# jorge-menjivar/tekken-rs

Hardware: AMD Instinct MI355X
Metric: input MB/s tokenized (whole node) (higher is better)
Workload: dtype u8

## Files before the change

include/tekken_hip.h:

```cpp
#ifndef TEKKEN_HIP_H
#define TEKKEN_HIP_H
#include <stddef.h>
#include <stdint.h>

#ifdef __cplusplus
extern "C" {
#endif

#define TK_OK 0
#define TK_ERR_INVALID_CONFIG (-1)
#define TK_ERR_RUNTIME (-2)
#define TK_ERR_INVALID_UTF8 (-3)
#define TK_ERR_NO_DEVICE (-4)
#define TK_ERR_INVALID_ARG (-5)
#define TK_ERR_IO (-6)
#define TK_ERR_JSON (-7)
#define TK_ERR_BASE64 (-8)
#define TK_ERR_TOKEN_NOT_FOUND (-9)
#define TK_ERR_SPECIAL_POLICY (-10)

#define TK_POLICY_IGNORE 0
#define TK_POLICY_KEEP 1
#define TK_POLICY_RAISE 2

typedef struct tk_ctx tk_ctx;


int tk_ctx_create(const uint8_t* token_bytes, const uint32_t* token_offsets, uint32_t n_ranks,
                  uint32_t num_special_tokens, uint32_t bos_id, uint32_t eos_id, int device_id,
                  tk_ctx** out_ctx);

void tk_ctx_destroy(tk_ctx* ctx);

const char* tk_last_error(const tk_ctx* ctx);

typedef struct tk_result {
    uint32_t* ids;
    uint64_t* offsets;
    uint64_t n_ids;
    uint64_t n_docs;
} tk_result;

int tk_encode_batch(tk_ctx* ctx, const uint8_t* bytes, const uint64_t* doc_offsets, uint64_t n_docs,
                    int add_bos, int add_eos, int validate_utf8, tk_result* out);
void tk_free_result(tk_result* r);

int tk_encode_one(tk_ctx* ctx, const uint8_t* text, uint64_t len, int add_bos, int add_eos, uint32_t* ids_out,
                  uint64_t ids_capacity, uint64_t* n_ids);
uint64_t tk_small_path_calls(const tk_ctx* ctx);
uint64_t tk_round_path_docs(const tk_ctx* ctx);
uint64_t tk_long_piece_records(const tk_ctx* ctx);
uint64_t tk_cut_chunks(const tk_ctx* ctx);
uint64_t tk_last_host_syncs(const tk_ctx* ctx);

int tk_ctx_set_memo(tk_ctx* ctx, int log2_entries, int policy);
int tk_ctx_memo_clear(tk_ctx* ctx);
int tk_memo_stats(const tk_ctx* ctx, uint64_t* lookups_last, uint64_t* hits_last, uint64_t* lookups_total, uint64_t* hits_total,
                  int* active_last);

int tk_ctx_set_pattern(tk_ctx* ctx, int mode);

void* tk_host_alloc(size_t bytes);
void tk_host_free(void* p);
int tk_encode_batch_pipelined(tk_ctx* ctx, const uint8_t* bytes, const uint64_t* doc_offsets, uint64_t n_docs,
                              int add_bos, int add_eos, uint64_t slice_bytes, uint32_t* ids_out, uint64_t ids_capacity,
                              uint64_t* offsets_out, uint64_t* n_ids);

int tk_encode_batch_device(tk_ctx* ctx, const void* d_bytes, const void* d_doc_offsets, uint64_t n_docs,
                           uint64_t n_bytes, int add_bos, int add_eos, void* hip_stream, void** d_ids,
                           void** d_out_offsets, uint64_t* n_ids);

#define TK_CHECK_OFFSETS 1
#define TK_CHECK_UTF8 2
int tk_encode_batch_device_ex(tk_ctx* ctx, const void* d_bytes, const void* d_doc_offsets, uint64_t n_docs, uint64_t n_bytes,
                              int add_bos, int add_eos, int checks, void* hip_stream, void** d_ids, void** d_out_offsets,
                              uint64_t* n_ids);

#define TK_SPANS_CHECK_COVER 4
#define TK_SPANS_CHECK_BYTES 8
int tk_token_spans_device(tk_ctx* ctx, const void* d_ids, const void* d_id_offsets, uint64_t n_docs, uint64_t n_ids,
                          const void* d_doc_offsets, const void* d_bytes, int checks, void* hip_stream, void** d_spans,
                          uint64_t* bad_doc);
int tk_encode_batch_device_spans(tk_ctx* ctx, const void* d_bytes, const void* d_doc_offsets, uint64_t n_docs, uint64_t n_bytes,
                                 int add_bos, int add_eos, int checks, void* hip_stream, void** d_ids, void** d_out_offsets,
                                 void** d_spans, uint64_t* n_ids, uint64_t* bad_doc);
int tk_encode_batch_spans(tk_ctx* ctx, const uint8_t* bytes, const uint64_t* doc_offsets, uint64_t n_docs, int add_bos,
                          int add_eos, int validate_utf8, int checks, tk_result* out, uint32_t** spans, uint64_t* bad_doc);
void tk_free_spans(uint32_t* spans);

#define TK_UNIT_BYTE 0
#define TK_UNIT_CHAR 1
#define TK_UNIT_UTF16 2
int tk_token_spans_units_device(tk_ctx* ctx, const void* d_ids, const void* d_id_offsets, uint64_t n_docs, uint64_t n_ids, int unit,
                                void* hip_stream, void** d_spans);
int tk_encode_batch_device_spans_units(tk_ctx* ctx, const void* d_bytes, const void* d_doc_offsets, uint64_t n_docs, uint64_t n_bytes,
                                       int add_bos, int add_eos, int checks, int unit, void* hip_stream, void** d_ids,
                                       void** d_out_offsets, void** d_spans, uint64_t* n_ids);
int tk_encode_batch_spans_units(tk_ctx* ctx, const uint8_t* bytes, const uint64_t* doc_offsets, uint64_t n_docs, int add_bos,
                                int add_eos, int validate_utf8, int unit, tk_result* out, uint32_t** spans);
int tk_spans_locate_device(tk_ctx* ctx, const void* d_spans, const void* d_id_offsets, uint64_t n_docs, uint64_t n_ids,
                           const void* d_ann_doc, const void* d_ann, uint64_t n_ann, void* hip_stream, void** d_tok_range,
                           uint64_t* bad_ann);

#define TK_DENSE_PAD_LEFT 1
#define TK_DENSE_TRUNC_LEFT 2
#define TK_DENSE_FIXED 4
#define TK_DENSE_I64 8
#define TK_DENSE_MASK 16
typedef struct tk_dense_opts { uint32_t max_length, multiple_of, pad_id, keep_head, keep_tail, flags; } tk_dense_opts;
typedef struct tk_dense { void* ids; uint8_t* mask; uint32_t* lengths; uint64_t n_docs, row_len, n_truncated; } tk_dense;
int tk_dense_from_ids_device(tk_ctx* ctx, const void* d_ids, const void* d_id_offsets, uint64_t n_docs, uint64_t n_ids,
                             const tk_dense_opts* opts, void* hip_stream, tk_dense* out);
int tk_encode_batch_device_dense(tk_ctx* ctx, const void* d_bytes, const void* d_doc_offsets, uint64_t n_docs, uint64_t n_bytes,
                                 int add_bos, int add_eos, int checks, const tk_dense_opts* opts, void* hip_stream,
                                 void** d_ids, void** d_out_offsets, uint64_t* n_ids, tk_dense* out);
int tk_encode_batch_dense(tk_ctx* ctx, const uint8_t* bytes, const uint64_t* doc_offsets, uint64_t n_docs, int add_bos,
                          int add_eos, int validate_utf8, const tk_dense_opts* opts, tk_dense* out);
void tk_free_dense(tk_dense* out);
int tk_ragged_from_dense_device(tk_ctx* ctx, const void* d_dense, uint64_t n_docs, uint64_t row_len, int flags,
                                const void* d_lengths, uint32_t pad_id, void* hip_stream, void** d_ids,
                                void** d_id_offsets, uint64_t* n_ids);

#define TK_SEQPACK_I64 1
#define TK_SEQPACK_POSITIONS 2
#define TK_SEQPACK_SEGMENTS 4
#define TK_SEQPACK_CU_SEQLENS 8
#define TK_SEQPACK_DROP_LAST 16
typedef struct tk_seqpack_opts { uint32_t seq_len, pad_id, flags; } tk_seqpack_opts;
typedef struct tk_seqpack { void *input_ids, *position_ids, *segment_ids; int32_t* cu_seqlens;
                            uint64_t n_rows, row_len, n_used, n_left, n_segments, max_seqlen; } tk_seqpack;
int tk_seqpack_from_ids_device(tk_ctx* ctx, const void* d_ids, const void* d_id_offsets, uint64_t n_docs, uint64_t n_ids,
                               const tk_seqpack_opts* opts, void* hip_stream, tk_seqpack* out);
int tk_encode_batch_device_seqpack(tk_ctx* ctx, const void* d_bytes, const void* d_doc_offsets, uint64_t n_docs, uint64_t n_bytes,
                                   int add_bos, int add_eos, int checks, const tk_seqpack_opts* opts, void* hip_stream,
                                   void** d_ids, void** d_out_offsets, uint64_t* n_ids, tk_seqpack* out);
int tk_encode_batch_seqpack(tk_ctx* ctx, const uint8_t* bytes, const uint64_t* doc_offsets, uint64_t n_docs, int add_bos, int add_eos,
// ... 172 lines not shown
```

tekken-rs_amd/__init__.py:

```python
import ctypes
import enum
import os
import subprocess

import numpy as np

_HERE = os.path.dirname(os.path.abspath(__file__))
LIB_PATH = os.environ.get("TK_HIP_LIB") or os.path.join(_HERE, "libtekken_hip.so")
INCLUDE_DIR = os.path.join(os.path.dirname(_HERE), "include")

TK_OK = 0
CHECK_OFFSETS, CHECK_UTF8 = 1, 2
SPANS_CHECK_COVER, SPANS_CHECK_BYTES = 4, 8
UNIT_BYTE, UNIT_CHAR, UNIT_UTF16 = 0, 1, 2
_UNITS = {"byte": UNIT_BYTE, "char": UNIT_CHAR, "utf16": UNIT_UTF16}
DENSE_PAD_LEFT, DENSE_TRUNC_LEFT, DENSE_FIXED, DENSE_I64, DENSE_MASK = 1, 2, 4, 8, 16
SEQPACK_I64, SEQPACK_POSITIONS, SEQPACK_SEGMENTS, SEQPACK_CU_SEQLENS, SEQPACK_DROP_LAST = 1, 2, 4, 8, 16
WINDOW_FIXED, WINDOW_I64, WINDOW_MASK, WINDOW_SPANS = 1, 2, 4, 8
CHECK_PARTS = 16
JOIN_NONE = 0xFFFFFFFF
PART_LABEL_CTRL, PART_LABEL_TEXT = 1, 2
JOIN_LABELS, JOIN_PART_INDEX = 1, 2
ROWFIT_I64, ROWFIT_POSITIONS, ROWFIT_SEGMENTS, ROWFIT_CU_SEQLENS, ROWFIT_LABELS, ROWFIT_DOC_START = 1, 2, 4, 8, 16, 32
REGROUP_ORDER_KEEP, REGROUP_ORDER_LENGTH, REGROUP_ORDER_SHUFFLE, REGROUP_ORDER_GROUPED = 0, 1, 2, 3
# ... 76 lines not shown

class _Join(ctypes.Structure):
    _fields_ = [("ids", ctypes.c_void_p), ("offsets", ctypes.c_void_p), ("labels", ctypes.c_void_p), ("part_index", ctypes.c_void_p),
                ("n_convs", ctypes.c_uint64), ("n_parts", ctypes.c_uint64), ("n_ids", ctypes.c_uint64), ("n_ctrl", ctypes.c_uint64),
                ("n_labelled", ctypes.c_uint64)]


class _RowfitOpts(ctypes.Structure):
    _fields_ = [("seq_len", ctypes.c_uint32), ("pad_id", ctypes.c_uint32), ("keep_tail", ctypes.c_uint32), ("flags", ctypes.c_uint32),
                ("ignore_index", ctypes.c_int32)]


class _Rowfit(ctypes.Structure):
    _fields_ = [("input_ids", ctypes.c_void_p), ("labels", ctypes.c_void_p), ("position_ids", ctypes.c_void_p), ("segment_ids", ctypes.c_void_p),
                ("cu_seqlens", ctypes.c_void_p), ("doc_start", ctypes.c_void_p), ("n_rows", ctypes.c_uint64), ("row_len", ctypes.c_uint64),
                ("n_segments", ctypes.c_uint64), ("max_seqlen", ctypes.c_uint64), ("n_truncated", ctypes.c_uint64), ("n_pad", ctypes.c_uint64)]


class _RegroupOpts(ctypes.Structure):
    _fields_ = [("max_tokens", ctypes.c_uint64), ("min_length", ctypes.c_uint32), ("max_length", ctypes.c_uint32), ("order", ctypes.c_uint32),
                ("seed", ctypes.c_uint32), ("window", ctypes.c_uint32), ("max_docs", ctypes.c_uint32), ("flags", ctypes.c_uint32)]


class _Regroup(ctypes.Structure):
    _fields_ = [("ids", ctypes.c_void_p), ("offsets", ctypes.c_void_p), ("labels", ctypes.c_void_p), ("perm", ctypes.c_void_p),
                ("batch_offsets", ctypes.c_void_p), ("batch_rowlen", ctypes.c_void_p), ("n_docs", ctypes.c_uint64), ("n_ids", ctypes.c_uint64),
                ("n_masked", ctypes.c_uint64), ("n_short", ctypes.c_uint64), ("n_long", ctypes.c_uint64), ("n_batches", ctypes.c_uint64),
                ("n_oversize", ctypes.c_uint64), ("n_batch_pad", ctypes.c_uint64)]


_LIB = None


def build(force=False):
    if force:
        subprocess.check_call(["make", "-s", "-C", _HERE, "clean"])
    subprocess.check_call(["make", "-s", "-j4", "-C", _HERE, "libtekken_hip.so"])
    return LIB_PATH


def lib():
    global _LIB
    if _LIB is not None:
        return _LIB
    if not os.path.exists(LIB_PATH):
        raise RuntimeError("libtekken_hip.so is missing: run `make -C tekken-rs_amd` (or __graft_entry__.build())")
    try:
        import torch
    except ImportError:
        pass
    L = ctypes.CDLL(LIB_PATH)
    vp, u8p, u32p, u64p = ctypes.c_void_p, ctypes.POINTER(ctypes.c_uint8), ctypes.POINTER(ctypes.c_uint32), ctypes.POINTER(ctypes.c_uint64)
    L.tk_ctx_create.restype = ctypes.c_int
    L.tk_ctx_create.argtypes = [u8p, u32p, ctypes.c_uint32, ctypes.c_uint32, ctypes.c_uint32, ctypes.c_uint32,
                                ctypes.c_int, ctypes.POINTER(vp)]
    L.tk_ctx_destroy.argtypes = [vp]
    L.tk_last_error.restype = ctypes.c_char_p
    L.tk_last_error.argtypes = [vp]
    L.tk_encode_batch.restype = ctypes.c_int
    L.tk_encode_batch.argtypes = [vp, u8p, u64p, ctypes.c_uint64, ctypes.c_int, ctypes.c_int, ctypes.c_int,
                                  ctypes.POINTER(_Result)]
    L.tk_free_result.argtypes = [ctypes.POINTER(_Result)]
    L.tk_encode_one.restype = ctypes.c_int
    L.tk_encode_one.argtypes = [vp, ctypes.c_char_p, ctypes.c_uint64, ctypes.c_int, ctypes.c_int, u32p, ctypes.c_uint64, u64p]
    L.tk_small_path_calls.restype = ctypes.c_uint64
    L.tk_small_path_calls.argtypes = [vp]
    L.tk_round_path_docs.restype = ctypes.c_uint64
    L.tk_round_path_docs.argtypes = [vp]
    L.tk_long_piece_records.restype = ctypes.c_uint64
    L.tk_long_piece_records.argtypes = [vp]
    if hasattr(L, "tk_ctx_set_memo"):
        L.tk_ctx_set_memo.restype = ctypes.c_int
        L.tk_ctx_set_memo.argtypes = [vp, ctypes.c_int, ctypes.c_int]
        L.tk_ctx_memo_clear.restype = ctypes.c_int
        L.tk_ctx_memo_clear.argtypes = [vp]
        L.tk_memo_stats.restype = ctypes.c_int
        L.tk_memo_stats.argtypes = [vp, u64p, u64p, u64p, u64p, ctypes.POINTER(ctypes.c_int)]
    if hasattr(L, "tk_last_host_syncs"):
        L.tk_last_host_syncs.restype = ctypes.c_uint64
        L.tk_last_host_syncs.argtypes = [vp]
    if hasattr(L, "tk_cut_chunks"):
        L.tk_cut_chunks.restype = ctypes.c_uint64
        L.tk_cut_chunks.argtypes = [vp]
    L.tk_encode_batch_device.restype = ctypes.c_int
    L.tk_encode_batch_device.argtypes = [vp, vp, vp, ctypes.c_uint64, ctypes.c_uint64, ctypes.c_int, ctypes.c_int, vp,
                                         ctypes.POINTER(vp), ctypes.POINTER(vp), ctypes.POINTER(ctypes.c_uint64)]
    L.tk_encode_batch_device_ex.restype = ctypes.c_int
    L.tk_encode_batch_device_ex.argtypes = [vp, vp, vp, ctypes.c_uint64, ctypes.c_uint64, ctypes.c_int, ctypes.c_int, ctypes.c_int, vp,
                                            ctypes.POINTER(vp), ctypes.POINTER(vp), ctypes.POINTER(ctypes.c_uint64)]
    L.tk_host_alloc.restype = ctypes.c_void_p
    L.tk_host_alloc.argtypes = [ctypes.c_size_t]
    L.tk_host_free.argtypes = [ctypes.c_void_p]
    L.tk_encode_batch_pipelined.restype = ctypes.c_int
    L.tk_encode_batch_pipelined.argtypes = [vp, u8p, u64p, ctypes.c_uint64, ctypes.c_int, ctypes.c_int, ctypes.c_uint64, u32p,
                                            ctypes.c_uint64, u64p, u64p]
    L.tk_ids18_bytes.restype = ctypes.c_uint64
    L.tk_ids18_bytes.argtypes = [ctypes.c_uint64]
    L.tk_pack_ids18_device.restype = ctypes.c_int
    L.tk_pack_ids18_device.argtypes = [vp, vp, ctypes.c_uint64, vp, vp]
    L.tk_unpack_ids18_device.restype = ctypes.c_int
    L.tk_unpack_ids18_device.argtypes = [vp, vp, ctypes.c_uint64, vp, vp]
    L.tk_ctx_set_pattern.restype = ctypes.c_int
    L.tk_ctx_set_pattern.argtypes = [vp, ctypes.c_int]
    L.tk_tokenizer_set_honour_pattern.restype = ctypes.c_int
    L.tk_tokenizer_set_honour_pattern.argtypes = [vp, ctypes.c_int]
    L.tk_ctx_set_special_tokens.restype = ctypes.c_int
    L.tk_ctx_set_special_tokens.argtypes = [vp, u8p, u32p, ctypes.c_uint32]
    L.tk_decode_batch.restype = ctypes.c_int
    L.tk_decode_batch.argtypes = [vp, u32p, u64p, ctypes.c_uint64, ctypes.c_int, ctypes.POINTER(_TextResult), u64p]
    L.tk_free_text_result.argtypes = [ctypes.POINTER(_TextResult)]
    L.tk_decode_batch_device.restype = ctypes.c_int
    L.tk_decode_batch_device.argtypes = [vp, vp, vp, ctypes.c_uint64, ctypes.c_uint64, ctypes.c_int, vp, ctypes.POINTER(vp),
                                         ctypes.POINTER(vp), u64p, u64p]
    L.tk_tokenizer_decode_batch.restype = ctypes.c_int
    L.tk_tokenizer_decode_batch.argtypes = [vp, u32p, u64p, ctypes.c_uint64, ctypes.c_int, ctypes.POINTER(_TextResult), u64p]
    L.tk_last_timing.restype = ctypes.c_int
    if hasattr(L, "tk_last_merge_ms"):
        L.tk_last_merge_ms.restype = ctypes.c_float
        L.tk_last_merge_ms.argtypes = [vp]
    L.tk_last_timing.argtypes = [vp, ctypes.POINTER(ctypes.c_float), ctypes.POINTER(ctypes.c_float)]
    L.tk_last_stats.restype = ctypes.c_int
    L.tk_last_stats.argtypes = [vp, u64p, u64p]
    L.tk_split_batch.restype = ctypes.c_int
    L.tk_split_batch.argtypes = [vp, u8p, u64p, ctypes.c_uint64, u8p]
    L.tk_tokenizer_from_file.restype = ctypes.c_int
    L.tk_tokenizer_from_file.argtypes = [ctypes.c_char_p, ctypes.c_int, ctypes.POINTER(vp)]
    L.tk_tokenizer_from_json.restype = ctypes.c_int
    L.tk_tokenizer_from_json.argtypes = [ctypes.c_char_p, ctypes.c_size_t, ctypes.c_int, ctypes.POINTER(vp)]
    L.tk_tokenizer_destroy.argtypes = [vp]
    L.tk_tokenizer_last_error.restype = ctypes.c_char_p
    L.tk_tokenizer_last_error.argtypes = [vp]
    L.tk_tokenizer_encode.restype = ctypes.c_int
    L.tk_tokenizer_encode.argtypes = [vp, ctypes.c_char_p, ctypes.c_size_t, ctypes.c_int, ctypes.c_int,
                                      ctypes.POINTER(u32p), ctypes.POINTER(ctypes.c_size_t)]
    L.tk_tokenizer_encode_batch.restype = ctypes.c_int
    L.tk_tokenizer_encode_batch.argtypes = [vp, u8p, u64p, ctypes.c_uint64, ctypes.c_int, ctypes.c_int,
                                            ctypes.POINTER(_Result)]
    L.tk_free_ids.argtypes = [u32p]
    L.tk_tokenizer_decode.restype = ctypes.c_int
    L.tk_tokenizer_decode.argtypes = [vp, u32p, ctypes.c_size_t, ctypes.c_int, ctypes.POINTER(ctypes.c_void_p),
                                      ctypes.POINTER(ctypes.c_size_t)]
    L.tk_free_text.argtypes = [ctypes.c_void_p]
    u64pp = ctypes.POINTER(ctypes.POINTER(ctypes.c_uint64))
    L.tk_free_offsets.argtypes = [ctypes.POINTER(ctypes.c_uint64)]
    L.tk_free_offsets.restype = None
    L.tk_tokenizer_decode_all.restype = ctypes.c_int
    L.tk_tokenizer_decode_all.argtypes = [vp, u32p, ctypes.c_size_t, ctypes.c_int, ctypes.POINTER(ctypes.c_void_p), u64pp,
                                          ctypes.POINTER(ctypes.c_size_t)]
    L.tk_tokenizer_vocab.restype = ctypes.c_int
    L.tk_tokenizer_vocab.argtypes = [vp, ctypes.POINTER(ctypes.c_void_p), u64pp, ctypes.POINTER(ctypes.c_size_t)]
    L.tk_tokenizer_vocab_size.restype = ctypes.c_uint32
    L.tk_tokenizer_vocab_size.argtypes = [vp]
    L.tk_tokenizer_num_special_tokens.restype = ctypes.c_uint32
    L.tk_tokenizer_num_special_tokens.argtypes = [vp]
    L.tk_tokenizer_version.restype = ctypes.c_char_p
    L.tk_tokenizer_version.argtypes = [vp]
    L.tk_tokenizer_control_token.restype = ctypes.c_int
    L.tk_tokenizer_control_token.argtypes = [vp, ctypes.c_char_p, u32p]
    L.tk_tokenizer_is_special.restype = ctypes.c_int
    L.tk_tokenizer_is_special.argtypes = [vp, ctypes.c_uint32]
    L.tk_tokenizer_is_byte.restype = ctypes.c_int
    L.tk_tokenizer_is_byte.argtypes = [vp, ctypes.c_uint32]
    L.tk_tokenizer_id_to_piece.restype = ctypes.c_int
    L.tk_tokenizer_id_to_piece.argtypes = [vp, ctypes.c_uint32, ctypes.POINTER(ctypes.c_void_p),
                                           ctypes.POINTER(ctypes.c_size_t)]
    L.tk_tokenizer_id_to_byte_piece.restype = ctypes.c_int
# ... 637 lines not shown
        return JoinResult.take(j)[1]

    def ragged_from_dense_device(self, d_dense_ptr, n_docs, row_len, flags=0, d_lengths_ptr=0, pad_id=0, stream=0):
        d_ids, d_oo, n = ctypes.c_void_p(), ctypes.c_void_p(), ctypes.c_uint64(0)
        self._call("tk_ragged_from_dense_device", ctypes.c_void_p(d_dense_ptr or None), n_docs, row_len, int(flags),
                   ctypes.c_void_p(d_lengths_ptr or None), int(pad_id), ctypes.c_void_p(stream),
                   ctypes.byref(d_ids), ctypes.byref(d_oo), ctypes.byref(n))
        return d_ids.value, d_oo.value, int(n.value)

    def encode_batch_device_views(self, d_bytes_ptr, d_offs_ptr, n_docs, n_bytes, add_bos=True, add_eos=True, stream=0):
        p_ids, p_oo, n = self.encode_batch_device(d_bytes_ptr, d_offs_ptr, n_docs, n_bytes, add_bos, add_eos, stream)
        return DeviceView(p_ids, n, "<i4"), DeviceView(p_oo, n_docs + 1, "<i8")

    def pack_ids18_device(self, d_ids_ptr, n_ids, d_packed_ptr, stream=0):
        rc = lib().tk_pack_ids18_device(self._h, ctypes.c_void_p(d_ids_ptr), n_ids, ctypes.c_void_p(d_packed_ptr), ctypes.c_void_p(stream))
        if rc != TK_OK:
            raise self._err(rc)

    def unpack_ids18_device(self, d_packed_ptr, n_ids, d_ids_ptr, stream=0):
        rc = lib().tk_unpack_ids18_device(self._h, ctypes.c_void_p(d_packed_ptr), n_ids, ctypes.c_void_p(d_ids_ptr), ctypes.c_void_p(stream))
        if rc != TK_OK:
            raise self._err(rc)

    def set_pattern(self, mode):
        rc = lib().tk_ctx_set_pattern(self._h, int(mode))
        if rc != TK_OK:
            raise self._err(rc)

    def set_special_tokens(self, strings):
        raw = [x.encode("utf-8") if isinstance(x, str) else bytes(x) for x in strings]
        offs = np.zeros(len(raw) + 1, np.uint32)
        offs[1:] = np.cumsum([len(x) for x in raw], dtype=np.uint64).astype(np.uint32)
        blob = np.frombuffer(b"".join(raw) or b"\0", dtype=np.uint8).copy()
        rc = lib().tk_ctx_set_special_tokens(self._h, _p(blob, ctypes.c_uint8), _p(offs, ctypes.c_uint32), len(raw))
        if rc != TK_OK:
            raise self._err(rc)

    def decode_batch(self, ids, offs, policy=SpecialTokenPolicy.Ignore):
        ids = np.ascontiguousarray(ids, dtype=np.uint32)
        offs = np.ascontiguousarray(offs, dtype=np.uint64)
        res = _TextResult()
        bad = ctypes.c_uint64(0)
        ibuf = ids if len(ids) else np.zeros(1, np.uint32)
        rc = lib().tk_decode_batch(self._h, _p(ibuf, ctypes.c_uint32), _p(offs, ctypes.c_uint64), len(offs) - 1, int(policy),
                                   ctypes.byref(res), ctypes.byref(bad))
        if rc != TK_OK:
            e = self._err(rc)
            e.bad_doc = int(bad.value)
            raise e
        n, D = int(res.n_bytes), int(res.n_docs)
        data = np.ctypeslib.as_array(res.bytes, shape=(max(n, 1),))[:n].copy()
        oo = np.ctypeslib.as_array(res.offsets, shape=(D + 1,)).copy()
        lib().tk_free_text_result(ctypes.byref(res))
        return data, oo

    def decode_docs(self, id_lists, policy=SpecialTokenPolicy.Ignore):
        offs = np.zeros(len(id_lists) + 1, np.uint64)
        if id_lists:
            offs[1:] = np.cumsum([len(x) for x in id_lists], dtype=np.uint64)
        ids = np.array([i for x in id_lists for i in x], dtype=np.uint32)
        data, oo = self.decode_batch(ids, offs, policy)
        raw = data.tobytes()
        return [raw[int(oo[d]):int(oo[d + 1])] for d in range(len(id_lists))]

    def decode_batch_device(self, d_ids_ptr, d_offs_ptr, n_docs, n_ids, policy=SpecialTokenPolicy.Ignore, stream=0):
        d_b, d_o, n, bad = ctypes.c_void_p(), ctypes.c_void_p(), ctypes.c_uint64(0), ctypes.c_uint64(0)
        rc = lib().tk_decode_batch_device(self._h, ctypes.c_void_p(d_ids_ptr), ctypes.c_void_p(d_offs_ptr), n_docs, n_ids,
                                          int(policy), ctypes.c_void_p(stream), ctypes.byref(d_b), ctypes.byref(d_o),
                                          ctypes.byref(n), ctypes.byref(bad))
        if rc != TK_OK:
            e = self._err(rc)
            e.bad_doc = int(bad.value)
            raise e
        return DeviceView(d_b.value, int(n.value), "|u1"), DeviceView(d_o.value, n_docs + 1, "<i8")

    def last_timing(self):
        a, b = ctypes.c_float(0), ctypes.c_float(0)
        lib().tk_last_timing(self._h, ctypes.byref(a), ctypes.byref(b))
        return {"pipeline_ms": a.value, "encode_kernel_ms": b.value, "merge_ms": float(lib().tk_last_merge_ms(self._h)) if hasattr(lib(), "tk_last_merge_ms") else 0.0}

    def last_stats(self):
        a, b = ctypes.c_uint64(0), ctypes.c_uint64(0)
        lib().tk_last_stats(self._h, ctypes.byref(a), ctypes.byref(b))
        return {"long_docs": int(a.value), "handed_back": int(b.value)}

    def split_docs(self, docs):
        data, offs = pack_docs(docs)
        n = int(offs[-1])
        out = np.zeros(max(n, 1), np.uint8)
        dbuf = data if n else np.zeros(1, np.uint8)
        rc = lib().tk_split_batch(self._h, _p(dbuf, ctypes.c_uint8), _p(offs, ctypes.c_uint64), len(docs),
                                  _p(out, ctypes.c_uint8))
        if rc != TK_OK:
            raise self._err(rc)
        res = []
        for d in range(len(docs)):
            a, b = int(offs[d]), int(offs[d + 1])
            res.append(np.nonzero(out[a:b])[0].tolist())
        return res


class Node:

    def __init__(self, token_bytes, num_special, bos_id, eos_id, devices=(0,)):
        toks = list(token_bytes)
        offs = np.zeros(len(toks) + 1, np.uint32)
        offs[1:] = np.cumsum([len(t) for t in toks], dtype=np.uint64).astype(np.uint32)
        blob = np.frombuffer(b"".join(toks) or b"\0", dtype=np.uint8)
        devs = (ctypes.c_int * len(devices))(*devices)
        h = ctypes.c_void_p()
        rc = lib().tk_node_create(_p(blob, ctypes.c_uint8), _p(offs, ctypes.c_uint32), len(toks), num_special, bos_id, eos_id,
                                  devs, len(devices), ctypes.byref(h))
        if rc != TK_OK:
            raise TokenizerError(rc, lib().tk_node_last_error(None).decode())
        self._h = h

    def close(self):
        if getattr(self, "_h", None):
            lib().tk_node_destroy(self._h)
            self._h = None

    def __del__(self):
        try:
            self.close()
        except Exception:
            pass

    def n_devices(self):
        return lib().tk_node_n_devices(self._h)

    def encode_batch(self, data, offs, add_bos=True, add_eos=True):
        data = np.ascontiguousarray(data, dtype=np.uint8)
        offs = np.ascontiguousarray(offs, dtype=np.uint64)
        res = _Result()
        dbuf = data if len(data) else np.zeros(1, np.uint8)
        rc = lib().tk_node_encode_batch(self._h, _p(dbuf, ctypes.c_uint8), _p(offs, ctypes.c_uint64), len(offs) - 1, int(add_bos),
                                        int(add_eos), ctypes.byref(res))
        if rc != TK_OK:
            raise TokenizerError(rc, lib().tk_node_last_error(self._h).decode())
        return _take_result(res)

    def encode_batch_into(self, data, offs, ids_out, offs_out, add_bos=True, add_eos=True):
        assert data.dtype == np.uint8 and offs.dtype == np.uint64 and ids_out.dtype == np.uint32 and offs_out.dtype == np.uint64
        assert len(offs_out) >= len(offs), "offs_out holds %d offsets, the call writes %d" % (len(offs_out), len(offs))
        for a in (data, offs, ids_out, offs_out):
            assert a.flags["C_CONTIGUOUS"], "tk_node_encode_batch_pinned wants contiguous buffers"
        n = ctypes.c_uint64(0)
        dbuf = data if len(data) else np.zeros(1, np.uint8)
        rc = lib().tk_node_encode_batch_pinned(self._h, _p(dbuf, ctypes.c_uint8), _p(offs, ctypes.c_uint64), len(offs) - 1, int(add_bos),
                                               int(add_eos), _p(ids_out, ctypes.c_uint32), len(ids_out), _p(offs_out, ctypes.c_uint64), ctypes.byref(n))
        if rc != TK_OK:
            raise TokenizerError(rc, lib().tk_node_last_error(self._h).decode())
        return int(n.value)

    def last_timing(self):
        a, b = ctypes.c_float(0), ctypes.c_float(0)
        lib().tk_node_last_timing(self._h, ctypes.byref(a), ctypes.byref(b))
        return {"kernels_ms_max": a.value, "gather_ms": b.value}

    def last_shards(self):
        n = self.n_devices()
        b, i = (ctypes.c_uint64 * n)(), (ctypes.c_uint64 * n)()
        lib().tk_node_last_shards(self._h, b, i, n)
        return list(b), list(i)


class _Pinned:
# ... 547 lines not shown
```

tekken-rs_amd/csrc/tk_capi.cpp:

```cpp
#include <unordered_map>

#include "tk_ctx.h"

static thread_local std::string g_tls_err;

void tk_set_tls_error(const std::string& e) { g_tls_err = e; }
const std::string& tk_get_tls_error() { return g_tls_err; }

namespace {

struct PinPool {
    std::mutex mu;
    std::unordered_map<void*, size_t> live;
    std::vector<std::pair<void*, size_t>> free_blocks;
    size_t free_bytes = 0;
    void* get(size_t bytes) {
        if (bytes == 0) bytes = 1;
        {
            std::lock_guard<std::mutex> lock(mu);
            size_t best = free_blocks.size();
            for (size_t i = 0; i < free_blocks.size(); ++i)
                if (free_blocks[i].second >= bytes && free_blocks[i].second <= 4 * bytes + (1u << 16) &&
                    (best == free_blocks.size() || free_blocks[i].second < free_blocks[best].second))
                    best = i;
// ... 29 lines not shown
                }
            }
        }
        (void)hipHostFree(p);
    }
};
PinPool g_pin_pool;

}

void* tk_pinned_get(size_t bytes) { return g_pin_pool.get(bytes); }
void tk_pinned_put(void* p) { g_pin_pool.put(p); }

int upload(tk_ctx* c, DevBuf& b, const void* src, size_t bytes) {
    TK_HIP(c, b.reserve(bytes ? bytes : 16));
    if (bytes) TK_HIP(c, hipMemcpy(b.p, src, bytes, hipMemcpyHostToDevice));
    return TK_OK;
}

int check_n_docs(tk_ctx* c, uint64_t n_docs) {
    if (n_docs >= 0xFFFFFFF0ull) { c->err = "too many documents in one batch"; return TK_ERR_INVALID_ARG; }
    return TK_OK;
}
int enter_device(tk_ctx* c, uint64_t n_docs) {
    int rc = check_n_docs(c, n_docs);
    if (rc != TK_OK) return rc;
    TK_HIP(c, hipSetDevice(c->device));
    return TK_OK;
}

static int copy_out_fail(tk_ctx* c, CopyOut* a, int n, const std::string& err) {
    for (int i = 0; i < n; ++i) { tk_pinned_put(a[i].host); a[i].host = nullptr; }
    c->err = err;
    return TK_ERR_RUNTIME;
}
int pinned_blocks(tk_ctx* c, CopyOut* a, int n) {
    bool ok = true;
    for (int i = 0; i < n; ++i)
        if (a[i].selected) ok = (a[i].host = tk_pinned_get(a[i].bytes)) != nullptr && ok;
    return ok ? TK_OK : copy_out_fail(c, a, n, "hipHostMalloc failed");
}
int copy_out(tk_ctx* c, CopyOut* a, int n, const char* what) {
    int rc = pinned_blocks(c, a, n);
    if (rc != TK_OK) return rc;
    hipError_t e = hipSuccess;
    for (int i = 0; i < n && e == hipSuccess; ++i)
        if (a[i].selected && a[i].dev && a[i].bytes) e = hipMemcpyAsync(a[i].host, a[i].dev, a[i].bytes, hipMemcpyDeviceToHost, c->stream);
    if (e == hipSuccess) e = hipStreamSynchronize(c->stream);
    return e == hipSuccess ? TK_OK : copy_out_fail(c, a, n, std::string(what) + " copy failed: " + hipGetErrorString(e));
}

int check_flags_and_args(tk_ctx* c, int checks, int known, bool null_arg) {
    if (checks & ~known) { c->err = "unknown check flag"; return TK_ERR_INVALID_ARG; }
    if (null_arg) { c->err = "null argument"; return TK_ERR_INVALID_ARG; }
    return TK_OK;
}
int scan_u32(tk_ctx* c, DevBuf& workspace, const uint32_t* counts, uint64_t n, uint64_t* offs, hipStream_t s) {
    TK_HIP(c, workspace.reserve(scan_workspace_bytes(n)));
    TK_HIP(c, tk_launch_scan(counts, n, offs, (uint64_t*)workspace.p, s));
    return TK_OK;
}
int encode_batch_for_layout(tk_ctx* c, const uint8_t* bytes, const uint64_t* doc_offsets, uint64_t n_docs, int add_bos, int add_eos,
                            int validate_utf8, DevBatch* dev, uint64_t* n_ids) {
    tk_result res;
    int rc = encode_batch(c, bytes, doc_offsets, n_docs, add_bos, add_eos, validate_utf8, &res, dev);
    if (rc != TK_OK) return rc;
    *n_ids = res.n_ids;
    tk_free_result(&res);
    return TK_OK;
}

static void read_knobs(TkKnobs& k) {
    if (const char* tl = getenv("TK_TAIL")) k.serial_tail = strcmp(tl, "serial") == 0;
    if (const char* dg = getenv("TK_DECODE_GROUPS")) k.no_decode_groups = strcmp(dg, "0") == 0;
    if (const char* gl = getenv("TK_DECODE_GROUP_LIMIT")) { const long long v = atoll(gl); if (v > 0 && v < 0x7FFFFF00ll) k.decode_group_limit = (uint32_t)v; }
    if (const char* fl = getenv("TK_FLAT_LONG")) k.no_flat_long = atoi(fl) == 0;
    if (const char* fl = getenv("TK_FLAT_LONG128")) k.no_flat_long128 = atoi(fl) == 0;
    if (const char* fl = getenv("TK_FLAT_CUT")) k.no_flat_cut = atoi(fl) == 0;
    if (const char* lm = getenv("TK_LONG_MIN")) k.long_min = (uint32_t)atoi(lm);
    if (const char* lz = getenv("TK_LONG_LAZY_MUL")) k.long_lazy_mul = (uint32_t)atoi(lz);
    if (const char* lf = getenv("TK_LONG_FORCE")) k.long_force = (uint32_t)atoi(lf);
    if (const char* ml = getenv("TK_MEMO_LOG2")) { const int v = atoi(ml); k.memo_log2 = v <= 0 ? 0u : (uint32_t)(v < 10 ? 10 : v > 26 ? 26 : v); }
    if (const char* mp = getenv("TK_MEMO_POLICY")) k.memo_policy = strcmp(mp, "always") == 0 ? 1 : 0;
    if (const char* pl = getenv("TK_PIPELINE"))
        k.pipeline_forced = strcmp(pl, "doc") == 0 ? 2 : strcmp(pl, "flat") == 0 ? 1 : 0;
}

extern "C" int tk_ctx_create(const uint8_t* token_bytes, const uint32_t* token_offsets, uint32_t n_ranks,
                             uint32_t num_special_tokens, uint32_t bos_id, uint32_t eos_id, int device_id,
                             tk_ctx** out_ctx) {
    if (!out_ctx) { g_tls_err = "out_ctx is NULL"; return TK_ERR_INVALID_ARG; }
    *out_ctx = nullptr;
    tk_ctx* c = new tk_ctx();
    std::string err;
    bool from_cache = false;
    int rc = tk_build_tables_cached(token_bytes, token_offsets, n_ranks, num_special_tokens, bos_id, eos_id, c->host, err, &from_cache);
    if (rc != TK_OK) { g_tls_err = err; delete c; return rc; }

    int n_dev = 0;
    hipError_t e = hipGetDeviceCount(&n_dev);
    if (e != hipSuccess || n_dev <= 0) {
        g_tls_err = "no HIP device available (the tokenization path has no CPU fallback)";
        delete c;
        return TK_ERR_NO_DEVICE;
    }
    if (device_id < 0 || device_id >= n_dev) {
        g_tls_err = "device_id out of range";
        delete c;
        return TK_ERR_INVALID_ARG;
    }
    c->device = device_id;
    auto fail = [&](int code) {
        g_tls_err = c->err;
        tk_ctx_destroy(c);
        return code;
    };
    auto fail_msg = [&](const char* msg) { c->err = msg; return fail(TK_ERR_RUNTIME); };
    if (hipSetDevice(device_id) != hipSuccess) return fail_msg("hipSetDevice failed");
    if (hipStreamCreateWithFlags(&c->stream.h, hipStreamNonBlocking) != hipSuccess) return fail_msg("hipStreamCreate failed");
    for (Event& ev : c->ev)
        if (hipEventCreate(&ev.h) != hipSuccess) return fail_msg("hipEventCreate failed");
    if (hipStreamCreateWithFlags(&c->stream_b.h, hipStreamNonBlocking) != hipSuccess) return fail_msg("hipStreamCreate failed");
    for (Event& ev : c->ev_b)
        if (hipEventCreateWithFlags(&ev.h, hipEventDisableTiming) != hipSuccess) return fail_msg("hipEventCreate failed");
    read_knobs(c->knobs);
    if (c->h_pin.alloc(TKC_PIN_WORDS * 4, hipHostMallocDefault) != hipSuccess) return fail_msg("hipHostMalloc failed");

    const TkHostTables& h = c->host;
    if (getenv("TK_DEBUG_LOG"))
        fprintf(stderr, "[tk] tables%s: KEY8 %u slots, KEY16 %u slots (hash mode %u, %llu keys, %llu in their second slot, %llu slots flagged), PAIR %u buckets (%llu pairs)\n",
                from_cache ? " (from cache)" : "", h.key8_mask + 1, h.key_mask + 1, h.key_hash_mode, (unsigned long long)h.n_key, (unsigned long long)h.n_key_second,
                (unsigned long long)h.n_key_spill_slots, h.pair_mask + 1, (unsigned long long)h.n_pairs);
    c->dview = h.host_view();
    auto up = [&](DevBuf& b, const auto& v, auto*& view) {
        if (rc == TK_OK && (rc = upload(c, b, v.data(), v.size() * sizeof(v[0]))) == TK_OK) view = (std::remove_reference_t<decltype(view)>)b.p;
    };
    TkTablesView& dv = c->dview;
    up(c->t_uc1, h.uc_stage1, dv.uc_stage1);    up(c->t_uc2, h.uc_stage2, dv.uc_stage2);
    up(c->t_uc2a, h.uc2_stage1, dv.uc2_stage1); up(c->t_uc2b, h.uc2_stage2, dv.uc2_stage2);
    up(c->t_key8, h.key8_tab, dv.key8_tab);     up(c->t_key, h.key_tab, dv.key_tab);
    up(c->t_long, h.long_tab, dv.long_tab);     up(c->t_pair, h.pair_tab, dv.pair_tab);
    up(c->t_pair2, h.pair2, dv.pair2);          up(c->t_pairf, h.pair_filter, dv.pair_filter);
    up(c->t_ucbmp, h.uc_bmp, dv.uc_bmp);        up(c->t_key64, h.key64_tab, dv.key64_tab);
    up(c->t_cutk2, h.cut_k2, dv.cut_k2);        up(c->t_cutg3, h.cut_g3, dv.cut_g3);
    up(c->t_blob, h.blob, dv.blob);
    if (rc != TK_OK || (rc = upload(c, c->t_offs, h.offs.data(), h.offs.size() * 4)) != TK_OK) return fail(rc);

    if (c->counters.reserve(TKC_DEVICE_WORDS * 4) != hipSuccess) return fail_msg("hipMalloc(counters) failed");
    uint32_t bad = 1;
    if (hipMemsetAsync(c->ctr(TKC_WORK), 0, TKC_DEVICE_WORDS * 4, c->stream) != hipSuccess ||
        tk_launch_wave_selftest(c->ctr(TKC_WORK), c->stream) != hipSuccess ||
        hipMemcpyAsync(&bad, c->ctr(TKC_WORK), 4, hipMemcpyDeviceToHost, c->stream) != hipSuccess ||
        hipStreamSynchronize(c->stream) != hipSuccess) {
        c->err = std::string("wave self-test launch failed: ") + hipGetErrorString(hipGetLastError());
        return fail(TK_ERR_RUNTIME);
    }
    if (bad != 0) {
        c->err = "wave primitive self-test failed on this device (mask " + std::to_string(bad) + ")";
        return fail(TK_ERR_RUNTIME);
    }
    *out_ctx = c;
    return TK_OK;
}

extern "C" void tk_ctx_destroy(tk_ctx* c) {
    if (!c) return;
    (void)hipSetDevice(c->device);
    delete c;
}

extern "C" int tk_ctx_set_pattern(tk_ctx* c, int mode) {
    TK_ENTRY(c);
    if (mode != 0 && mode != 1) { c->err = "pattern mode must be 0 (hard-coded pattern) or 1 (tekken.json pattern)"; return TK_ERR_INVALID_ARG; }
    c->pattern = mode;
    return TK_OK;
}

extern "C" const char* tk_last_error(const tk_ctx* c) { return c ? c->err.c_str() : g_tls_err.c_str(); }

const TkHostTables* tk_ctx_host_tables(const tk_ctx* c) { return c ? &c->host : nullptr; }

extern "C" const uint32_t* tk_debug_marks(const tk_ctx* c) { return c ? c->dbg_mark.p : nullptr; }

extern "C" float tk_last_merge_ms(const tk_ctx* c) { return c ? c->merge_ms : 0.f; }

extern "C" int tk_last_timing(const tk_ctx* c, float* pipeline_ms, float* encode_kernel_ms) {
    if (!c) return TK_ERR_INVALID_ARG;
    if (pipeline_ms) *pipeline_ms = c->pipeline_ms;
    if (encode_kernel_ms) *encode_kernel_ms = c->encode_ms;
    return TK_OK;
}

extern "C" int tk_ctx_set_memo(tk_ctx* c, int log2_entries, int policy) {
    TK_ENTRY(c);
    if (log2_entries != 0 && (log2_entries < 10 || log2_entries > 26)) { c->err = "memo size: log2_entries must be 0 (off) or 10..26"; return TK_ERR_INVALID_ARG; }
    if (policy != 0 && policy != 1) { c->err = "memo policy must be 0 (adaptive) or 1 (always)"; return TK_ERR_INVALID_ARG; }
    c->knobs.memo_log2 = (uint32_t)log2_entries;
    c->knobs.memo_policy = policy;
    c->memo_pause = 0; c->memo_low_streak = 0;
    if (log2_entries == 0) {
        TK_HIP(c, hipSetDevice(c->device));
        TK_HIP(c, hipDeviceSynchronize());
        c->t_memo.release();
        c->t_memo_log.release();
        c->memo_have_log2 = 0;
    }
    return TK_OK;
}
extern "C" int tk_ctx_memo_clear(tk_ctx* c) {
    TK_ENTRY(c);
    c->memo_have_log2 = 0;
    c->memo_pause = 0; c->memo_low_streak = 0;
    return TK_OK;
}
extern "C" int tk_memo_stats(const tk_ctx* c, uint64_t* lookups_last, uint64_t* hits_last, uint64_t* lookups_total, uint64_t* hits_total, int* active_last) {
    if (!c) return TK_ERR_INVALID_ARG;
    if (lookups_last) *lookups_last = c->memo_lookups_last;
    if (hits_last) *hits_last = c->memo_hits_last;
    if (lookups_total) *lookups_total = c->memo_lookups_total;
    if (hits_total) *hits_total = c->memo_hits_total;
    if (active_last) *active_last = c->memo_active_last ? 1 : 0;
    return TK_OK;
}

extern "C" uint64_t tk_small_path_calls(const tk_ctx* c) { return c ? c->n_small_calls : 0; }
extern "C" uint64_t tk_round_path_docs(const tk_ctx* c) { return c ? c->n_round_docs : 0; }
extern "C" uint64_t tk_long_piece_records(const tk_ctx* c) { return c ? c->n_long_recs : 0; }
extern "C" uint64_t tk_cut_chunks(const tk_ctx* c) { return c ? c->n_cut_chunks : 0; }
extern "C" uint64_t tk_last_host_syncs(const tk_ctx* c) { return c ? c->host_syncs : 0; }

extern "C" int tk_last_stats(const tk_ctx* c, uint64_t* n_long_docs, uint64_t* reserved) {
    if (!c) return TK_ERR_INVALID_ARG;
    if (n_long_docs) *n_long_docs = c->n_long_docs;
    if (reserved) *reserved = c->n_flagged;
    return TK_OK;
}

extern "C" int tk_ctx_set_special_tokens(tk_ctx* c, const uint8_t* blob, const uint32_t* offs, uint32_t n) {
    TK_ENTRY(c);
    if (!offs || n != c->host.num_special || (!blob && n && offs[n])) {
        c->err = "special token strings: need exactly num_special_tokens entries";
        return TK_ERR_INVALID_ARG;
    }
    TK_HIP(c, hipSetDevice(c->device));
    int rc;
    if ((rc = upload(c, c->t_spblob, blob, n ? offs[n] : 0)) || (rc = upload(c, c->t_spoffs, offs, ((size_t)n + 1) * 4))) return rc;
    c->have_specials = true;
    return TK_OK;
}
```

tekken-rs_amd/csrc/tk_counters.h:

```cpp
#ifndef TK_COUNTERS_H
#define TK_COUNTERS_H

enum TkCounter {
    TKC_WORK = 0,
    TKC_DEFERRED = 1,
    TKC_INVALID = 2,
    TKC_DEFER_MAXLEN = 3,
    TKC_HANDED_BACK = 4,
    TKC_PASS2_SPARE = 5,
    TKC_TOTAL = 6,
    TKC_PACK_BAD = 8,
    TKC_LONG_LIST = 9,
    TKC_LONG_JOBS = 10,
    TKC_LONG_RECS = 11,
    TKC_CUT_CHUNKS = 12,
    TKC_TODO = 13,
    TKC_TODO_MAXLEN = 14,
    TKC_LATE = 15,
    TKC_LONG_CTL = 16,
    TKC_LONG_CTL_HI = 17,
    TKC_LONG_CTL_CAP = 18,
    TKC_CUT_CTL = 19,
    TKC_CUT_CTL_HI = 20,
    TKC_MEMO_HITS = 24,
    TKC_NARROW_LEFT = 25,

    TKC_CLEARED = 16,
    TKC_EARLY_WORDS = 16,
    TKC_FINAL_WORDS = 28,
    TKC_DEVICE_WORDS = 32,
    TKC_EARLY_MIRROR = 32,
    TKC_PIN_WORDS = 64
};
#define TKC_CTL(word) ((int)(word) - (int)TKC_LONG_CTL)
#define TKC_OVERFLOW 0xDEADu

static_assert(TKC_LONG_CTL >= TKC_CLEARED && TKC_CUT_CTL_HI < TKC_MEMO_HITS, "the control words lie outside what the pre-pass clears");
static_assert(TKC_TODO_MAXLEN < TKC_EARLY_WORDS && TKC_NARROW_LEFT < TKC_FINAL_WORDS && TKC_FINAL_WORDS <= TKC_DEVICE_WORDS, "copies hold what the host reads");
static_assert(TKC_FINAL_WORDS <= TKC_EARLY_MIRROR && TKC_EARLY_MIRROR + TKC_EARLY_WORDS <= TKC_PIN_WORDS, "both copies fit h_pin, apart");
static_assert(TKC_LONG_CTL_CAP == TKC_LONG_CTL + 2 && TKC_CUT_CTL == TKC_LONG_CTL + 3 && TKC_CUT_CTL_HI == TKC_CUT_CTL + 1, "one block of control words");

#endif
```

tekken-rs_amd/csrc/tk_ctx.h:

```cpp
#ifndef TK_CTX_H
#define TK_CTX_H
#include <hip/hip_runtime.h>
#include <stdint.h>
#include <stdio.h>
#include <stdlib.h>
#include <string.h>

#include <mutex>
#include <string>
#include <utility>
#include <vector>

#include "../../include/tekken_hip.h"
#include "tekkenizer.hpp"
#include "tk_counters.h"
#include "tk_engine.h"
#include "tk_kernels.h"
#include "tk_tables.h"

struct DevBuf {
    void* p = nullptr;
    size_t cap = 0;
    DevBuf() = default;
    DevBuf(DevBuf&& o) noexcept : p(o.p), cap(o.cap) { o.p = nullptr; o.cap = 0; }
    DevBuf& operator=(DevBuf&& o) noexcept { std::swap(p, o.p); std::swap(cap, o.cap); return *this; }
    ~DevBuf() { release(); }
    hipError_t reserve(size_t bytes) {
        if (bytes <= cap) return hipSuccess;
        release();
        size_t want = bytes + bytes / 8 + 256;
        hipError_t e = hipMalloc(&p, want);
        if (e == hipSuccess) cap = want;
        return e;
    }
    void release() {
        if (p) (void)hipFree(p);
        p = nullptr; cap = 0;
    }
};

struct NoCopy { NoCopy() = default; NoCopy(const NoCopy&) = delete; NoCopy& operator=(const NoCopy&) = delete; };

template <class T> struct PinBuf : NoCopy {
    T* p = nullptr;
    ~PinBuf() { release(); }
    hipError_t alloc(size_t bytes, unsigned flags) { release(); return hipHostMalloc((void**)&p, bytes, flags); }
    void release() { if (p) (void)hipHostFree(p); p = nullptr; }
    operator T*() const { return p; }
};

template <class H, hipError_t (*Destroy)(H)> struct Handle : NoCopy {
    H h = nullptr;
    ~Handle() { if (h) (void)Destroy(h); }
    operator H() const { return h; }
};
typedef Handle<hipStream_t, hipStreamDestroy> Stream;
typedef Handle<hipEvent_t, hipEventDestroy> Event;

struct TkKnobs {
    bool serial_tail = false;
    bool no_decode_groups = false;
    uint32_t decode_group_limit = 0x7FFFFF00u;
    bool no_flat_long = false;
    bool no_flat_long128 = false;
    bool no_flat_cut = false;
    uint32_t long_min = 256;
    uint32_t long_lazy_mul = 0;
    uint32_t long_force = 0;
    uint32_t memo_log2 = 24;
    int memo_policy = 0;
    int pipeline_forced = 0;
};
struct TkCallKnobs {
    bool log = false;
    bool marks = false;
    bool skip_pass2 = false;
    int memo_log_log2 = 0;
    int ablate = 0;
};

struct SpansBufs { DevBuf spans, err; };
struct UnitsBufs { DevBuf table, spans, err, range, next, range_err; };
struct DenseBufs { DevBuf ids, mask, len, stat, rids, roffs, rlens; };
struct SeqpackBufs { DevBuf ids, pos, seg, cu, stat, flags, aflags, fpos, apos, starts, aligned, bsum; };
struct JoinBufs { DevBuf ids, offs, labels, pidx, stat, has, cb, start, plocal, bsum, in_ctrl, in_flags, in_conv; };
struct WindowBufs { DevBuf ids, mask, spans, len, doc, start, dw, dw_next, cnt, bsum, stat; };
struct RowfitBufs {
    DevBuf ids, lab, pos, seg, cu, dstart, stat, e, nz, E, nzp, ja, jb, row, open, segno, padf, padp, bsum;
    Event ev[5];
    float ms[3] = {0.f, 0.f, 0.f};
    float ms_chain = 0.f;
};
struct RegroupBufs {
    DevBuf ids, offs, lab, perm, bo, brl, stat, flag, fpos, kept, key[2], val[3], hist, hpos, len, src, pyr, ja, jb, row, open, bmax, bsum;
    Event ev[6];
    float ms[4] = {0.f, 0.f, 0.f, 0.f};
};

struct tk_ctx {
    int device = 0;
    std::mutex mu;
    std::string err;
    TkKnobs knobs;
    TkCallKnobs call;
    TkHostTables host;
    TkTablesView dview;
    Stream stream, stream_b, s_in, s_out;
    Event ev[5];
    Event ev_b[3];
    Event ev_in[2], ev_out[2];
    DevBuf t_uc1, t_uc2, t_key8, t_key, t_long, t_pair, t_pair2, t_pairf, t_blob, t_offs, t_spblob, t_spoffs, t_uc2a, t_uc2b;
    DevBuf t_key64;
    DevBuf t_cutk2, t_cutg3, t_ucbmp;
    int pattern = 0;
    bool have_specials = false;
    DevBuf dec_lens, dec_bytes, dec_offs, dec_bits, dec_err, dec_in_ids, dec_in_offs, dec_hi, dec_glens, dec_goffs;
    DevBuf t_inline, t_len8;
    SpansBufs spans;
    UnitsBufs units;
    DenseBufs dense;
    SeqpackBufs seqpack;
    JoinBufs join;
    WindowBufs window;
    RowfitBufs rowfit;
    RegroupBufs regroup;
    DevBuf staging, counts, out_ids, out_offs, block_sums, defer_list, scratch, in_bytes, in_offs, dbg;
    DevBuf counters;
    PinBuf<uint32_t> h_pin;
    PinBuf<uint32_t> dbg_mark;
    DevBuf long_jobs;
    DevBuf long_list;
    DevBuf f_first, f_tmp, f_lstart, f_flags, f_todo, f_miss, f_mcnt, f_mpfx, f_wfirst, f_info;
    DevBuf f_long;
    DevBuf f_cut;
    DevBuf f_late;
    DevBuf scratch_rec;
    void* long_ctl_ptr = nullptr;
    uint32_t long_ctl_cap = 0;
    void* cut_ctl_ptr = nullptr;
    bool use_flat = true;
    uint64_t n_flagged = 0, n_long_docs = 0;
    uint64_t n_round_docs = 0;
    uint64_t n_long_recs = 0;
    uint64_t n_cut_chunks = 0;
    uint32_t host_syncs = 0;
    float pipeline_ms = 0.f, encode_ms = 0.f, merge_ms = 0.f;
    DevBuf in_bytes2, in_offs2, out_ids2, out_offs2;
    PinBuf<uint64_t> h_offs_stage[2];
    uint64_t h_offs_cap = 0;
    PinBuf<uint8_t> hs_in;
    PinBuf<uint32_t> hs_out;
    void* ds_in = nullptr, *ds_out = nullptr;
    DevBuf s_offs;
    uint64_t n_small_calls = 0;
    bool small_ready = false;
    DevBuf t_memo, t_memo_log;
    uint32_t memo_have_log2 = 0;
    uint32_t memo_epoch = 0;
    uint32_t memo_low_streak = 0, memo_pause = 0;
    bool memo_active_last = false;
    uint64_t memo_hits_last = 0, memo_lookups_last = 0, memo_hits_total = 0, memo_lookups_total = 0;

    uint32_t* ctr(int word) const { return (uint32_t*)counters.p + word; }
};

#define TK_SMALL_IDS_CAP (TK_SMALL_MAX_BYTES + 2 * TK_SMALL_MAX_DOCS)
#define TK_SMALL_OUT_OFFS_WORD (TK_SMALL_IDS_CAP)
#define TK_SMALL_STATUS_WORD (TK_SMALL_OUT_OFFS_WORD + 2 * (TK_SMALL_MAX_DOCS + 1) + 2)

#define TK_HIP(ctx, call)                                                                          \
    do {                                                                                           \
        hipError_t _e = (call);                                                                    \
        if (_e != hipSuccess) { (ctx)->err = std::string(#call) + ": " + hipGetErrorString(_e); return TK_ERR_RUNTIME; } \
    } while (0)

#define TK_ENTRY(c)                                                                                \
    if (!(c)) return TK_ERR_INVALID_ARG;                                                           \
    std::lock_guard<std::mutex> lock((c)->mu)

#pragma GCC visibility push(hidden)
int upload(tk_ctx* c, DevBuf& b, const void* src, size_t bytes);
int check_n_docs(tk_ctx* c, uint64_t n_docs);
int enter_device(tk_ctx* c, uint64_t n_docs);
struct CopyOut { const void* dev; size_t bytes; void* host; bool selected = true; };
int pinned_blocks(tk_ctx* c, CopyOut* a, int n);
int copy_out(tk_ctx* c, CopyOut* a, int n, const char* what);
#define TK_LAYOUT_MAX_ROW 0x7FFFFFFFull
#define TK_LAYOUT_MAX_ELEMS (1ull << 36)
int check_flags_and_args(tk_ctx* c, int checks, int known, bool null_arg);
static inline size_t scan_workspace_bytes(uint64_t n) { return (n / 2048 + 4) * 8; }
int scan_u32(tk_ctx* c, DevBuf& workspace, const uint32_t* counts, uint64_t n, uint64_t* offs, hipStream_t s);
int run_pipeline(tk_ctx* c, const uint8_t* d_bytes, const uint64_t* d_offs, uint64_t n_docs, uint64_t n_bytes, int add_bos,
                 int add_eos, hipStream_t s, uint64_t* n_ids);
TkEncodeArgs encode_args(tk_ctx* c, const uint8_t* d_bytes, const uint64_t* d_offs, uint64_t n_docs, int add_bos, int add_eos);
int check_offsets(tk_ctx* c, const uint64_t* doc_offsets, uint64_t n_docs);
int encode_device_checked(tk_ctx* c, const void* d_bytes, const void* d_doc_offsets, uint64_t n_docs, uint64_t n_bytes, int add_bos,
                          int add_eos, int checks, void* hip_stream, void** d_ids, void** d_out_offsets, uint64_t* n_ids);
struct DevBatch {
    const uint8_t* bytes = nullptr; const uint64_t* doc_offs = nullptr;
    const uint32_t* ids = nullptr;  const uint64_t* id_offs = nullptr;
};
int encode_batch(tk_ctx* c, const uint8_t* bytes, const uint64_t* doc_offsets, uint64_t n_docs, int add_bos, int add_eos,
                 int validate_utf8, tk_result* out, DevBatch* dev);
int encode_batch_for_layout(tk_ctx* c, const uint8_t* bytes, const uint64_t* doc_offsets, uint64_t n_docs, int add_bos, int add_eos,
                            int validate_utf8, DevBatch* dev, uint64_t* n_ids);
int encode_parts_device_join(tk_ctx* c, const void* d_bytes, const void* d_doc_offsets, uint64_t n_parts, uint64_t n_bytes,
                             const void* d_part_ctrl, const void* d_part_flags, const void* d_conv_offsets, uint64_t n_convs,
                             int checks, const tk_join_opts* opts, void* hip_stream, tk_join* out);
int token_tables(tk_ctx* c);
template <class A> static inline void token_args(const tk_ctx* c, A& a) {
    a.tok_blob = (const uint8_t*)c->t_blob.p; a.tok_offs = (const uint32_t*)c->t_offs.p;
    a.tok_inline = (const uint8_t*)c->t_inline.p; a.tok_len8 = (const uint8_t*)c->t_len8.p;
    a.n_ranks = c->host.n_ranks; a.num_special = c->host.num_special;
}
int run_spans(tk_ctx* c, const uint32_t* d_ids, const uint64_t* d_id_offs, uint64_t n_docs, uint64_t n_ids, const uint64_t* d_doc_offs,
              const uint8_t* d_bytes, int checks, hipStream_t s, uint64_t* bad_doc, DevBuf* into = nullptr);
int doc_of_id(tk_ctx* c, const uint64_t* d_id_offs, uint64_t n_docs, uint64_t idx, uint64_t* out);
// ... 4 lines not shown
```

tekken-rs_amd/csrc/tk_flat.hip:

```cpp
#include <hip/hip_runtime.h>
#include <stdint.h>
#include <stdlib.h>

#include "tk_kernels.h"
#include "tk_wave_hip.h"
#include "tk_flat_impl.h"
#include "tk_flat_tail_impl.h"

#define TKF_BLOCK 256
#ifndef TKF_OCC
#define TKF_OCC __attribute__((amdgpu_waves_per_eu(7, 7)))
#endif

__global__ __launch_bounds__(TKF_BLOCK) void tk_flat_firstdoc_kernel(const uint64_t* __restrict__ doc_offs, uint64_t n_docs,
                                                                      uint64_t n_chunks, uint32_t* __restrict__ first_doc,
                                                                      uint32_t* __restrict__ flags, uint32_t* __restrict__ holes,
                                                                      uint32_t* __restrict__ counters16) {
    tkf_firstdoc_body((uint64_t)blockIdx.x * TKF_BLOCK + threadIdx.x, doc_offs, n_docs, n_chunks, first_doc, flags, holes, counters16);
}

template <int DBG, int MODE, int PAT = 0, int MEMO = 1>
__device__ __forceinline__ void tk_flat_kernel_body(const TkFlatArgs& a, uint32_t* lds_all) {
    const int lane = wv_lane();
    const uint32_t wv = (uint32_t)__builtin_amdgcn_readfirstlane((int)(threadIdx.x >> 6));
// ... 22 lines not shown
__global__ __launch_bounds__(TKF_BLOCK) TKF_OCC void tk_flat_mode1_kernel(TkFlatArgs a) {
    __shared__ uint32_t lds_all[(TKF_BLOCK / 64) * TKF_LDS_WORDS];
    tk_flat_kernel_body<0, 1>(a, lds_all);
}

__global__ __launch_bounds__(TKF_BLOCK) TKF_OCC void tk_flat_json_kernel(TkFlatArgs a) {
    __shared__ uint32_t lds_all[(TKF_BLOCK / 64) * TKF_LDS_WORDS];
    if (a.t.key_hash_mode == 0u) tk_flat_kernel_body<0, 0, 1>(a, lds_all);
    else tk_flat_kernel_body<0, 1, 1>(a, lds_all);
}

__global__ __launch_bounds__(TKF_BLOCK) TKF_OCC void tk_flat_split_kernel(TkFlatArgs a) {
    __shared__ uint32_t lds_all[(TKF_BLOCK / 64) * TKF_LDS_WORDS];
    if (a.t.key_hash_mode == 0u) tk_flat_kernel_body<1, 0>(a, lds_all);
    else tk_flat_kernel_body<1, 1>(a, lds_all);
}

template <int DBG>
__device__ __forceinline__ void tk_flat_cut_body(const TkFlatArgs& a, uint32_t* lds_all) {
    const uint32_t n = *a.cut_count;
    if (n == 0u) return;
    const int lane = wv_lane();
    const uint32_t wv = (uint32_t)__builtin_amdgcn_readfirstlane((int)(threadIdx.x >> 6));
    uint32_t* lds = lds_all + wv * TKF_LDS_WORDS_CUT;
    tk_flat_init_lds(a, lds, lane);
    const uint64_t n_waves = (uint64_t)gridDim.x * (TKF_BLOCK / 64);
    for (uint64_t i = (uint64_t)blockIdx.x * (TKF_BLOCK / 64) + wv; i < n; i += n_waves) {
        const uint64_t c = (uint64_t)__builtin_amdgcn_readfirstlane((int)a.cut_list[i]);
        if (a.t.key_hash_mode == 0u) tk_flat_chunk<DBG, 0, 0, 1>(a, c, lane, lds);
        else tk_flat_chunk<DBG, 1, 0, 1>(a, c, lane, lds);
    }
    tk_flat_flush_memo_hits(a, lds, lane);
}
__global__ __launch_bounds__(TKF_BLOCK) void tk_flat_cut_kernel(TkFlatArgs a) {
    __shared__ uint32_t lds_all[(TKF_BLOCK / 64) * TKF_LDS_WORDS_CUT];
    tk_flat_cut_body<0>(a, lds_all);
}
__global__ __launch_bounds__(TKF_BLOCK) void tk_flat_cut_split_kernel(TkFlatArgs a) {
    __shared__ uint32_t lds_all[(TKF_BLOCK / 64) * TKF_LDS_WORDS_CUT];
    tk_flat_cut_body<1>(a, lds_all);
}

__global__ __launch_bounds__(TKF_BLOCK) void tk_merge_wavefirst_kernel(const uint64_t* __restrict__ prefix, uint64_t n_chunks,
                                                                        uint32_t* __restrict__ wave_first,
                                                                        uint32_t* __restrict__ wave_first_wide,
                                                                        uint32_t* __restrict__ narrow_left_out) {
    tkf_wavefirst_body((uint64_t)blockIdx.x * TKF_BLOCK + threadIdx.x, prefix, n_chunks, wave_first, wave_first_wide, narrow_left_out);
}

template <int THREADS, uint32_t WORDS = TK_PAIRF_WORDS>
TK_DEV void tk_merge_load_filter(const TkFlatArgs& a, uint32_t* filt) {
    const tk_u32x4* src = reinterpret_cast<const tk_u32x4*>(a.t.pair_filter);
    for (uint32_t i = threadIdx.x; i < WORDS / 4; i += THREADS) reinterpret_cast<tk_u32x4*>(filt)[i] = src[i];
    __syncthreads();
}

#ifndef TKM_BLOCK
#define TKM_BLOCK 1024
#endif
#ifndef TKM_WIDE_BLOCK
#define TKM_WIDE_BLOCK 1024
#endif
#ifndef TKM_FILTER
#define TKM_FILTER 1
#endif
#define TKM_FWORDS (TKM_FILTER ? TK_PAIRF_WORDS : 0u)
#define TKM_LDS_BYTES ((TKM_FWORDS + (TKM_BLOCK / 64) * TKM_LDS_WORDS(16)) * 4)
#ifndef TKM_WIDE_FILTER
#define TKM_WIDE_FILTER 0
#endif
#define TKM_WIDE_FWORDS (TKM_WIDE_FILTER ? TK_PAIRF_WORDS : 0u)
#define TKM_WIDE_LDS_BYTES ((TKM_WIDE_FWORDS + (TKM_WIDE_BLOCK / 64) * TKM_LDS_WORDS(32)) * 4)
__global__ __launch_bounds__(TKM_BLOCK) void tk_merge_kernel(TkFlatArgs a) {
    extern __shared__ __attribute__((aligned(16))) uint32_t wlds[];
    if (TKM_FILTER) tk_merge_load_filter<TKM_BLOCK, TK_PAIRF_WORDS>(a, wlds);
    const uint64_t wave = (uint64_t)blockIdx.x * (TKM_BLOCK / 64) + (threadIdx.x >> 6);
    const uint64_t n_waves = (uint64_t)gridDim.x * (TKM_BLOCK / 64);
    const uint64_t total = a.miss_prefix[2 * a.n_chunks];
    uint32_t* mlds = wlds + TKM_FWORDS + (threadIdx.x >> 6) * TKM_LDS_WORDS(16);
    TkMemoLog ml;
    ml.base = a.memo_log ? a.memo_log + wave * a.memo_log_per_wave : nullptr;
    ml.n = 0u;
    ml.cap = a.memo_log && wave < a.memo_log_waves ? a.memo_log_per_wave : 0u;
    for (uint64_t w = wave; w * 64 < total; w += n_waves) tk_merge_wave<false>(a, w, wv_lane(), mlds, TKM_FILTER ? wlds : nullptr, a.memo_log ? &ml : nullptr);
    if (a.memo_log && wave < a.memo_log_waves && wv_lane() == 0) a.memo_log_counts[wave] = ml.n;
}

__global__ __launch_bounds__(TKF_BLOCK) void tk_memo_commit_kernel(tk_memo_entry* __restrict__ tab, const tk_memo_entry* __restrict__ log,
                                                                    const uint32_t* __restrict__ counts, uint32_t per_wave, uint32_t n_waves,
                                                                    uint32_t key_hash_mode, uint32_t mask) {
    const uint32_t n = per_wave * n_waves;
    for (uint32_t i = blockIdx.x * TKF_BLOCK + threadIdx.x; i < n; i += gridDim.x * TKF_BLOCK)
        if (tk_memo_log_live(counts, per_wave, i)) tk_memo_commit_one(tab, log, i, key_hash_mode, mask);
}

__global__ __launch_bounds__(TKM_WIDE_BLOCK) void tk_merge_wide_kernel(TkFlatArgs a) {
    extern __shared__ __attribute__((aligned(16))) uint32_t wlds[];
    if (TKM_WIDE_FILTER) tk_merge_load_filter<TKM_WIDE_BLOCK, TKM_WIDE_FWORDS>(a, wlds);
    const uint32_t* wfilt = TKM_WIDE_FILTER ? wlds : nullptr;
    const uint64_t wave = (uint64_t)blockIdx.x * (TKM_WIDE_BLOCK / 64) + (threadIdx.x >> 6);
    const uint64_t n_waves = (uint64_t)gridDim.x * (TKM_WIDE_BLOCK / 64);
    const uint64_t n2 = a.miss_prefix[3 * a.n_chunks] - a.miss_prefix[2 * a.n_chunks];
    const uint64_t n3 = a.miss_prefix[4 * a.n_chunks] - a.miss_prefix[3 * a.n_chunks];
    const uint64_t w2 = (n2 + 63) / 64, w3 = (n3 + 63) / 64;
    uint32_t* mlds = wlds + TKM_WIDE_FWORDS + (threadIdx.x >> 6) * TKM_LDS_WORDS(32);
    for (uint64_t w = wave; w < w2; w += n_waves) tk_merge_wave<true>(a, w, wv_lane(), mlds, wfilt);
    if (w3 == 0) return;
    __syncthreads();
    if (((threadIdx.x >> 6) & 1u) == 0u) {
        const uint64_t ew = wave >> 1, n_ew = n_waves >> 1;
        for (uint64_t w = ew; w < w3; w += n_ew) tk_merge_wave_long3(a, w, wv_lane(), mlds, wfilt);
    }
}

__global__ __launch_bounds__(TKF_BLOCK) void tk_flat_todo_kernel(const uint32_t* __restrict__ flags, const uint64_t* __restrict__ doc_offs,
                                                                  uint64_t n_docs, uint32_t* __restrict__ todo,
                                                                  uint32_t* __restrict__ n_todo, uint32_t* __restrict__ maxlen) {
    tkf_todo_body((uint64_t)blockIdx.x * TKF_BLOCK + threadIdx.x, wv_lane(), flags, doc_offs, n_docs, todo, n_todo, maxlen);
}

__global__ __launch_bounds__(TKF_BLOCK) void tk_flat_counts_kernel(const uint64_t* __restrict__ doc_offs, uint64_t n_docs,
                                                                    uint64_t n_bytes, uint64_t n_chunks,
                                                                    const uint64_t* __restrict__ P,
                                                                    const uint32_t* __restrict__ lstart,
                                                                    const uint32_t* __restrict__ flags,
                                                                    const uint32_t* __restrict__ holes, uint32_t extra,
                                                                    uint32_t* __restrict__ counts,
                                                                    TkFlatDocInfo* __restrict__ info, int final_pass,
                                                                    uint32_t* __restrict__ n_flagged) {
    tkf_counts_body((uint64_t)blockIdx.x * TKF_BLOCK + threadIdx.x, wv_lane(), doc_offs, n_docs, n_bytes, n_chunks, P, lstart, flags, holes,
                    extra, counts, info, final_pass, n_flagged);
}

__global__ __launch_bounds__(TKF_BLOCK) void tk_flat_assemble_kernel(TkFlatAssembleArgs a) {
    tkf_assemble_waves(a, (uint64_t)blockIdx.x * (TKF_BLOCK / 64) + (threadIdx.x >> 6), (uint64_t)gridDim.x * (TKF_BLOCK / 64), wv_lane());
}

static uint32_t tkf_blocks(uint64_t n_threads) { return (uint32_t)((n_threads + TKF_BLOCK - 1) / TKF_BLOCK); }

hipError_t tk_launch_flat_firstdoc(const uint64_t* doc_offs, uint64_t n_docs, uint64_t n_chunks, uint32_t* first_doc,
                                   uint32_t* flags, uint32_t* holes, uint32_t* counters16, hipStream_t s) {
    hipLaunchKernelGGL(tk_flat_firstdoc_kernel, dim3(tkf_blocks(n_docs + 32)), dim3(TKF_BLOCK), 0, s, doc_offs, n_docs,
                       n_chunks, first_doc, flags, holes, counters16);
    return hipGetLastError();
}

hipError_t tk_launch_flat(const TkFlatArgs& a, hipStream_t s) {
    if (a.n_chunks == 0) return hipSuccess;
    uint64_t blocks = (a.n_chunks + (TKF_BLOCK / 64) - 1) / (TKF_BLOCK / 64);
    static uint64_t cap_dev[64] = {0};
    int dev = 0;
    (void)hipGetDevice(&dev);
    uint64_t& cap = cap_dev[dev & 63];
    if (cap == 0) {
        int cus = 256;
        (void)hipDeviceGetAttribute(&cus, hipDeviceAttributeMultiprocessorCount, dev);
        int per_cu = 0;
        if (hipOccupancyMaxActiveBlocksPerMultiprocessor(&per_cu, tk_flat_kernel, TKF_BLOCK, 0) != hipSuccess || per_cu <= 0) per_cu = 4;
        cap = (uint64_t)cus * (uint64_t)per_cu;
        if (const char* e = getenv("TK_FLAT_BLOCKS")) cap = (uint64_t)atoll(e);
        if (cap == 0) cap = 1280;
    }
    if (blocks > cap) blocks = cap;
    if (a.pattern == 1) hipLaunchKernelGGL(tk_flat_json_kernel, dim3((uint32_t)blocks), dim3(TKF_BLOCK), 0, s, a);
    else if (a.dbg_ablate || a.dbg_starts) hipLaunchKernelGGL(tk_flat_split_kernel, dim3((uint32_t)blocks), dim3(TKF_BLOCK), 0, s, a);
    else if (a.t.key_hash_mode == 0u && a.memo_tab && a.memo_probe) hipLaunchKernelGGL(tk_flat_memo_kernel, dim3((uint32_t)blocks), dim3(TKF_BLOCK), 0, s, a);
    else if (a.t.key_hash_mode == 0u) hipLaunchKernelGGL(tk_flat_kernel, dim3((uint32_t)blocks), dim3(TKF_BLOCK), 0, s, a);
// ... 138 lines not shown
```

tekken-rs_amd/csrc/tk_flat_args.h:

```cpp
#ifndef TK_FLAT_ARGS_H
#define TK_FLAT_ARGS_H
#include <stdint.h>

#include "tk_counters.h"
#include "tk_tables.h"

#define TKF_W 32
#define TKF_REGION (64 * TKF_W)
#define TKF_HL 32
#define TKF_HR 64
#define TKF_COMMIT (TKF_REGION - TKF_HL - TKF_HR)
#define TKF_LONGCAP 256u
#define TKF_STRIDE (TKF_COMMIT + 64 + TKF_LONGCAP)
#define TKF_OWN (TKF_COMMIT + TKF_HR)
#define TKF_MISSOFF0 0u
#define TKF_MISSOFF1 (TKF_OWN / 2u)
#define TKF_MISSOFF2 (TKF_MISSOFF1 + (TKF_OWN + 8u) / 9u)
#define TKF_MISSOFF3 (TKF_MISSOFF2 + (TKF_OWN + 16u) / 17u)
#define TKF_MISSCAP ((TKF_MISSOFF3 + (TKF_OWN + 32u) / 33u + 7u) & ~7u)
#define TKF_POSBITS 11
#define TKF_REC(pos, len, slot) ((pos) | ((len) << TKF_POSBITS) | ((slot) << (TKF_POSBITS + 7)))
#define TKF_REC_POS(rec) ((rec) & ((1u << TKF_POSBITS) - 1u))
#define TKF_REC_LEN(rec) (((rec) >> TKF_POSBITS) & 127u)
#define TKF_REC_SLOT(rec) ((rec) >> (TKF_POSBITS + 7))
#define TKF_HOLE 0xFFFFFFFFu

struct TkFlatLongRec {
    uint64_t pos;
    uint32_t chunk;
    uint32_t slot;
    uint32_t len;
    uint32_t reserved;
};

#define TKF_LREC_FRAG 0x80000000u

struct TkFlatArgs {
    const uint8_t* bytes;
    const uint64_t* doc_offs;
    uint64_t n_docs, n_bytes, n_chunks;
    const uint32_t* first_doc;
    uint32_t* tmp;
    uint32_t* kcount;
    uint32_t* lstart;
    uint32_t* miss_list;
    uint32_t* miss_count;
    const uint64_t* miss_prefix;
    uint32_t* wave_first;
    uint32_t* wave_first_wide;
    uint32_t* holes;
    uint32_t* flags;
    TkFlatLongRec* long_recs;
    uint32_t* long_count;
    uint32_t long_cap;
    int long_merge128;
    const uint32_t* long_ctl;
    uint32_t* cut_list;
    const uint32_t* cut_count;
    uint32_t* late_list;
    uint32_t* late_count;
    tk_memo_entry* memo_tab;
    uint32_t memo_mask;
    int memo_probe;
    uint32_t memo_epoch;
    uint32_t* memo_hits;
    tk_memo_entry* memo_log;
    uint32_t* memo_log_counts;
    uint32_t memo_log_per_wave, memo_log_waves;
    uint8_t* dbg_starts;
    int pattern;
    int dbg_ablate;
    TkTablesView t;
};

#endif
```

tekken-rs_amd/csrc/tk_flat_impl.h:

```cpp
#ifndef TK_FLAT_IMPL_H
#define TK_FLAT_IMPL_H
#include <stdint.h>

#include "tk_encode_impl.h"
#include "tk_flat_args.h"

#define TKF_WM 0xFFFFFFFFu
#define TKF_LOGW 5
#define TKF_TOPBIT 0x80000000u
#define TKF_NHL (TKF_HL / TKF_W)
#ifndef TKF_LISTCAP
#define TKF_LISTCAP 1056
#endif
#define TKF_MAXPIECES (TKF_LISTCAP - 2)

#define TKF_L_LIST 0
#define TKF_L_DS (TKF_L_LIST + TKF_LISTCAP / 2)
#define TKF_L_PS (TKF_L_DS + 64)
#define TKF_L_PFX (TKF_L_PS + 64)
#define TKF_L_BAD (TKF_L_PFX + 64)
#define TKF_L_BPFX (TKF_L_BAD + 64)
#define TKF_WALKOFF 192
#define TKF_WALKCAP (2 * (TKF_LISTCAP / 2 - TKF_WALKOFF))
#define TKF_L_CL TKF_L_LIST
// ... 256 lines not shown
    if (neutral) {
        for (;;) {
            const uint32_t nxt = LW | (P1(LW) & neut);
            const bool grew = tkf_any(nxt & ~LW);
            LW = nxt;
            if (!grew) break;
        }
        uint32_t UE = m.UP & ~N1(mWd);
        for (;;) {
            const uint32_t nxt = UE | (N1(UE) & m.UP);
            const bool grew = tkf_any(nxt & ~UE);
            UE = nxt;
            if (!grew) break;
        }
        psC = CS & ((m.UP & P1(LW)) | (UE & P1(neut)));
    } else {
        psC = CS & m.UP & P1(LW);
    }
    const uint32_t psL = (Wst & P1(mN | NL | X)) | psC;
    const uint32_t psO = Oe & ~P1(Oe) & ~P1(SP);
    const uint32_t psN = mN & CS;
    const uint32_t SPR = mS & ~ABS;
    const uint32_t cont = SPR & P1(SPR);
    uint32_t Z = NL & SPR;
    {
        uint32_t C = tkf_shr(cont, 1);
        int k = 1;
        while (tkf_any(C) && tkf_any(Z)) {
            Z |= tkf_shr_any(Z, k, lane) & C;
            C &= tkf_shr_any(C, k, lane);
            k *= 2;
        }
    }
    uint32_t last = SPR & ~tkf_shr(cont, 1) & ~Z & nDE;
    if (u8) {
        last = (last & CS) | N1(last & U8C);
        last = (last & CS) | N1(last & U8C);
        last = (last & CS) | N1(last & U8C);
        last &= CS;
    }
    const uint32_t psS = (SPR & ~cont) | (tkf_shl(Z, 1) & cont & ~Z) | last;
#undef P1
#undef N1
    *SPR_out = SPR;
    *cont_out = cont;
    return psL | psN | psO | psS | after_abs | DS;
}

TK_DEV void tk_flat_init_lds(const TkFlatArgs& a, uint32_t* lds, int lane) {
    if (lane == 63) {
        const uint64_t b8 = (uint64_t)reinterpret_cast<uintptr_t>(a.t.key8_tab), b16 = (uint64_t)reinterpret_cast<uintptr_t>(a.t.key_tab);
        lds[TKF_L_CONST + 0] = a.t.key8_mask;
        lds[TKF_L_CONST + 1] = a.t.key_mask;
        lds[TKF_L_CONST + 2] = (uint32_t)b8; lds[TKF_L_CONST + 3] = (uint32_t)(b8 >> 32);
        lds[TKF_L_CONST + 4] = (uint32_t)b16; lds[TKF_L_CONST + 5] = (uint32_t)(b16 >> 32);
        const uint64_t lc = (uint64_t)reinterpret_cast<uintptr_t>(a.long_ctl);
        lds[TKF_L_CONST + 6] = (uint32_t)lc; lds[TKF_L_CONST + 7] = (uint32_t)(lc >> 32);
    }
    if (lane >= 1 && lane <= 16) {
        for (int q = 0; q < 4; ++q) {
            const int keep = lane - 4 * q;
            lds[TKF_L_KM + 4 * lane + q] = keep >= 4 ? 0xFFFFFFFFu : keep <= 0 ? 0u : ((1u << (8 * keep)) - 1u);
        }
    }
    if (lane == 0) {
        const uint64_t mb = a.memo_probe ? (uint64_t)reinterpret_cast<uintptr_t>(a.memo_tab) : 0ull;
        lds[TKF_L_MEMO + 0] = (uint32_t)mb; lds[TKF_L_MEMO + 1] = (uint32_t)(mb >> 32);
        lds[TKF_L_MEMO + 2] = a.memo_mask;
        lds[TKF_L_MEMO + 3] = 0u;
    }
    wv_lds_sync();
}

TK_DEV void tk_flat_flush_memo_hits(const TkFlatArgs& a, uint32_t* lds, int lane) {
    if (a.memo_tab && a.memo_hits) {
        wv_lds_sync();
        const uint32_t v = lds[TKF_L_MEMO + 3];
        if (lane == 0 && v != 0u) wv_atomic_add(a.memo_hits, v);
    }
}

TK_DEV uint32_t tkf_lowmask32(int n) { return n >= 32 ? 0xFFFFFFFFu : ((1u << n) - 1u); }

#ifdef TK_ABLATE
#define TKF_ABL(a, bit) (DBG && ((a).dbg_ablate & (bit)))
#else
#define TKF_ABL(a, bit) false
#endif

template <int DBG, int MODE, int PAT = 0, int CUT = 0, int MEMO = 1>
TK_DEV bool tk_flat_chunk(const TkFlatArgs& a, uint64_t c, int lane, uint32_t* lds) {
    const TkTablesView& t = a.t;
    const int64_t n = (int64_t)a.n_bytes;
    const int64_t c0 = (int64_t)c * TKF_COMMIT, r0 = c0 - TKF_HL, r1 = r0 + TKF_REGION;
    const int64_t c1 = c0 + TKF_COMMIT < n ? c0 + TKF_COMMIT : n;
    const int ca = TKF_HL, cb = (int)(c1 - r0);
    uint16_t* list = reinterpret_cast<uint16_t*>(lds + TKF_L_LIST);

    uint32_t x[TKF_W / 4];
    for (int k = 0; k < TKF_W / 4; ++k) x[k] = 0u;
    {
        const uint8_t* bytes = WV_KARGS(TkFlatArgs, a).bytes;
        const int64_t g = r0 + TKF_W * lane;
        if (g >= 0 && g + TKF_W <= n) {
            for (int k = 0; k < TKF_W / 16; ++k) wv_load16(bytes + g + 16 * k, x + 4 * k);
        } else if (g + TKF_W > 0 && g < n) {
            for (int k = 0; k < TKF_W; ++k) {
                const int64_t q = g + k;
                if (q >= 0 && q < n) x[k >> 2] |= (uint32_t)bytes[q] << (8 * (k & 3));
            }
        }
    }
    {
        uint32_t* txt = lds + TKF_L_TXT + (TKF_W / 4) * lane;
        for (int k = 0; k < TKF_W / 4; ++k) txt[k] = x[k];
        if (lane == 0) for (int k = 0; k < 4; ++k) lds[TKF_L_TXT + TKF_REGION / 4 + k] = 0u;
    }
    uint32_t nextb = 0;
    if (CUT && r1 < n) nextb = (uint32_t)a.bytes[r1];
    TkfClass m = tkf_classify(x);
    uint32_t walk = m.LEAD;
    if (!PAT && tkf_any(m.F2 | m.F3)) {
        m.L |= m.F2 | m.F3 | tkf_shl(m.F2 | m.F3, 1) | tkf_shl(m.F3, 2);
        walk &= ~(m.F2 | m.F3);
    }
    if (tkf_any(walk)) {
        uint32_t* cl = lds + TKF_L_CL;
        cl[lane] = 0u; cl[64 + lane] = 0u; cl[128 + lane] = 0u;
        if (PAT) { cl[192 + lane] = 0u; cl[256 + lane] = 0u; cl[320 + lane] = 0u; }
        if (lane == 0) {
            uint32_t pad = 0u;
            for (int k = 0; k < 4; ++k)
                if (r1 + k < n) pad |= (uint32_t)a.bytes[r1 + k] << (8 * k);
            lds[TKF_L_TXT + TKF_REGION / 4] = pad;
        }
        wv_lds_sync();
        bool nmb = false;
        uint32_t w = walk;
        auto decode = [&](int i, uint32_t* clen_out) -> uint32_t {
            const uint32_t p = (uint32_t)TKF_W * (uint32_t)lane + (uint32_t)i;
            const uint32_t* tw = lds + TKF_L_TXT + (p >> 2);
            const uint32_t v4 = wv_alignbyte(tw[1], tw[0], p & 3u);
            const uint32_t b0 = v4 & 0xFFu, b1 = (v4 >> 8) & 0xFFu, b2 = (v4 >> 16) & 0xFFu, b3 = v4 >> 24;
            uint32_t cp = 0xFFFFFFFFu, clen = 1;
            if (b0 < 0xE0u) {
                if ((b1 & 0xC0u) == 0x80u) { cp = ((b0 & 0x1Fu) << 6) | (b1 & 0x3Fu); clen = 2; }
            } else if (b0 < 0xF0u) {
                if ((b1 & 0xC0u) == 0x80u && (b2 & 0xC0u) == 0x80u) {
                    cp = ((b0 & 0x0Fu) << 12) | ((b1 & 0x3Fu) << 6) | (b2 & 0x3Fu); clen = 3;
                }
            } else if (b0 < 0xF8u) {
                if ((b1 & 0xC0u) == 0x80u && (b2 & 0xC0u) == 0x80u && (b3 & 0xC0u) == 0x80u) {
                    cp = ((b0 & 0x07u) << 18) | ((b1 & 0x3Fu) << 12) | ((b2 & 0x3Fu) << 6) | (b3 & 0x3Fu); clen = 4;
                }
            }
            *clen_out = clen;
            return cp;
        };
        auto mark = [&](int i, uint32_t clen, uint32_t cls, uint32_t extra) {
            if (PAT && extra) {
                const uint64_t xb = (uint64_t)((1u << clen) - 1u) << i;
                wv_lds_or(cl + (2u + extra) * 64u + (uint32_t)lane, (uint32_t)(xb & TKF_WM));
                if ((xb >> TKF_W) && lane < 63) wv_lds_or(cl + (2u + extra) * 64u + (uint32_t)lane + 1u, (uint32_t)(xb >> TKF_W));
            }
            if (cls != TK_CLS_O) {
                const uint64_t bits = (uint64_t)((1u << clen) - 1u) << i;
// ... 38 lines not shown
                        }
                        const uint32_t q = cp < 0x10000u ? cp : 0u;
                        uint32_t cw = t.uc_bmp[q >> 4];
                        uint32_t cls = (cw >> (2u * (q & 15u))) & 3u;
                        if (cp >= 0x10000u) cls = cp == 0xFFFFFFFFu ? (uint32_t)TK_CLS_O : tk_uc_class(t, cp);
                        if (cls != TK_CLS_O) {
                            const uint32_t wi = p >> TKF_LOGW, sh = p & (TKF_W - 1);
                            const uint64_t bits = (uint64_t)((1u << clen) - 1u) << sh;
                            wv_lds_or(cl + (cls - 1u) * 64u + wi, (uint32_t)(bits & TKF_WM));
                            if ((bits >> TKF_W) && wi < 63u) wv_lds_or(cl + (cls - 1u) * 64u + wi + 1u, (uint32_t)(bits >> TKF_W));
                            if (cls == TK_CLS_N) nmb = true;
                        }
                    }
                }
            }
        }
        while (!dealt && wv_ballot(w != 0u)) {
            if (w) {
                if (PAT) {
                    const int i = __builtin_ctz(w);
                    w &= w - 1u;
                    uint32_t clen;
                    const uint32_t cp = decode(i, &clen);
                    uint32_t cls = TK_CLS_O, extra = 0;
                    if (cp != 0xFFFFFFFFu) {
                        const uint32_t c2 = tk_uc_class2(t, cp);
                        cls = c2 == 1u || c2 == 2u ? TK_CLS_L : c2 == 5u ? TK_CLS_N : c2 == 6u ? TK_CLS_S : TK_CLS_O;
                        extra = c2 == 1u ? 1u : c2 == 3u ? 2u : c2 == 4u ? 3u : 0u;
                    }
                    mark(i, clen, cls, extra);
                } else {
                    const int i0 = __builtin_ctz(w);
                    w &= w - 1u;
                    const bool two = w != 0u;
                    const int i1 = two ? __builtin_ctz(w) : i0;
                    w &= w - 1u;
                    uint32_t l0, l1;
                    const uint32_t cp0 = decode(i0, &l0), cp1 = decode(i1, &l1);
                    const uint32_t q0 = cp0 < 0x10000u ? cp0 : 0u, q1 = cp1 < 0x10000u ? cp1 : 0u;
                    uint32_t w0 = t.uc_bmp[q0 >> 4], w1 = t.uc_bmp[q1 >> 4];
                    WV_PIN(w0); WV_PIN(w1);
                    uint32_t c0 = (w0 >> (2u * (q0 & 15u))) & 3u, c1 = (w1 >> (2u * (q1 & 15u))) & 3u;
                    if (cp0 >= 0x10000u) c0 = cp0 == 0xFFFFFFFFu ? (uint32_t)TK_CLS_O : tk_uc_class(t, cp0);
                    if (cp1 >= 0x10000u) c1 = cp1 == 0xFFFFFFFFu ? (uint32_t)TK_CLS_O : tk_uc_class(t, cp1);
                    mark(i0, l0, c0, 0u);
                    if (two) mark(i1, l1, c1, 0u);
                }
            }
        }
        wv_lds_sync();
        m.L |= cl[lane];
        m.N |= cl[64 + lane];
        m.S |= cl[128 + lane];
        m.nmb = wv_ballot(nmb) != 0ull;
        if (PAT) {
            m.UP |= cl[192 + lane];
            m.X = cl[256 + lane];
            m.M = cl[320 + lane];
        }
    }
    if (TKF_ABL(a, 16)) {
        const uint32_t v = m.L + m.N + m.S + m.NL + m.SP + m.AP + m.HI + m.STMD + m.RV + m.E + m.LL;
        if (lane == 0) {
            a.kcount[c] = v == 0xFFFFFFFFu ? 1u : 0u;
            for (int k = 0; k < 4; ++k) a.miss_count[k * a.n_chunks + c] = 0u;
        }
        return false;
    }

    lds[TKF_L_DS + lane] = 0u;
    lds[TKF_L_BAD + lane] = 0u;
    wv_lds_sync();
    const uint64_t fd = WV_KARGS(TkFlatArgs, a).first_doc[c];
    bool starts_at_r1 = false;
    {
        const auto& ka = WV_KARGS(TkFlatArgs, a);
        for (uint64_t base = fd;; base += 64) {
            const uint64_t d = base + (uint64_t)lane;
            int64_t s = INT64_MAX;
            if (d <= ka.n_docs) s = (int64_t)ka.doc_offs[d];
            const bool in = s < r1;
            if (in) wv_lds_or(lds + TKF_L_DS + ((s - r0) >> TKF_LOGW), 1u << ((s - r0) & (TKF_W - 1)));
            if (s == r1) starts_at_r1 = true;
            if (wv_ballot(in) != ~0ull) break;
        }
        starts_at_r1 = wv_ballot(starts_at_r1) != 0ull;
    }
    wv_lds_sync();
    const uint32_t DS = lds[TKF_L_DS + lane];

    uint32_t SPR, cont;
    uint32_t PS = PAT ? tkf_rules_json(m, DS, lane, &SPR, &cont) : tkf_rules(m, DS, lane, &SPR, &cont);
    if (TKF_ABL(a, 8)) {
        if (lane == 0) {
            a.kcount[c] = (PS + SPR + cont) == 0xFFFFFFFFu ? 1u : 0u;
            for (int k = 0; k < 4; ++k) a.miss_count[k * a.n_chunks + c] = 0u;
        }
        return false;
    }
    if (!CUT && !PAT) {
        const uint64_t Zm = wv_ballot(PS == 0u) & ~(((uint64_t)1 << TKF_NHL) - 1ull);
        if (Zm & (Zm >> 1)) {
            const uint64_t lc = (uint64_t)wv_first(lds[TKF_L_CONST + 6]) | ((uint64_t)wv_first(lds[TKF_L_CONST + 7]) << 32);
            if (lc != 0ull) {
                const uint32_t* ctl = reinterpret_cast<const uint32_t*>(wv_global_ptr(lc));
                const uint64_t lp = (uint64_t)wv_first(ctl[TKC_CTL(TKC_CUT_CTL)]) | ((uint64_t)wv_first(ctl[TKC_CTL(TKC_CUT_CTL_HI)]) << 32);
                if (lp != 0ull) {
                    if (lane == 0) {
                        const uint32_t q = wv_atomic_add(const_cast<uint32_t*>(ctl) + TKC_CTL(TKC_CUT_CHUNKS), 1u);
                        reinterpret_cast<uint32_t*>(const_cast<uint8_t*>(wv_global_ptr(lp)))[q] = (uint32_t)c;
                    }
                    return true;
                }
            }
        }
    }
    uint32_t commit_mask = (uint32_t)(lane - TKF_NHL) < (uint32_t)(TKF_COMMIT / TKF_W) ? TKF_WM : 0u;
    if (cb != TKF_HL + TKF_COMMIT)
        commit_mask = (tkf_lowmask32(cb - TKF_W * lane < 0 ? 0 : cb - TKF_W * lane) & ~tkf_lowmask32(ca - TKF_W * lane < 0 ? 0 : ca - TKF_W * lane)) & TKF_WM;
    if (DBG && a.dbg_starts) {
        for (int k = 0; k < TKF_W; ++k)
            if ((commit_mask >> k) & 1u) a.dbg_starts[r0 + TKF_W * lane + k] = (PS >> k) & 1u;
    }

    uint32_t BAD = 0;
    {
        const uint32_t d0 = wv_readlane(DS, 0);
        const uint32_t n0 = wv_readlane(m.N | (m.U8C & ~(m.U8C + 1u)), 0);
        const uint32_t l0 = wv_readlane((PAT ? (m.NL | m.SL) : m.NL) | (m.U8C & ~(m.U8C + 1u)), 0);
        const bool covered = n0 == TKF_WM || l0 == TKF_WM;
        if (r0 > 0 && d0 == 0u && covered && lane == TKF_NHL) BAD |= 1u;
        if (PAT) {
            const uint32_t lead_cont = m.U8C & ~(m.U8C + 1u);
            const uint32_t wd = m.L | m.X | m.M, om = (TKF_WM & ~(m.L | m.X | m.N | m.S));
            bool cov2 = wv_readlane(wd | lead_cont, 0) == TKF_WM || wv_readlane(om | m.NL | m.SL | lead_cont, 0) == TKF_WM;
            if (r0 > 0 && d0 == 0u && cov2 && lane == TKF_NHL) BAD |= 1u;
        }
        const uint32_t top = wv_readlane(SPR, 63);
        if (r1 < n && (top & TKF_TOPBIT) && !starts_at_r1) {
            const uint32_t nz = ~cont & TKF_WM;
            const uint64_t NZ = wv_ballot(nz != 0u);
            int f = 0;
            if (NZ) {
                const int tl = tk_msb64(NZ);
                const uint32_t w = wv_readlane(nz, tl);
                f = TKF_W * tl + (31 - __builtin_clz(w));
            }
            if (f < cb) {
                const int at = f > ca ? f : ca;
                if (lane == (at >> TKF_LOGW)) BAD |= 1u << (at & (TKF_W - 1));
            }
        }
    }

    uint32_t own_mask = commit_mask;
    uint32_t FS = 0;
    if (CUT) {
        const uint32_t R1 = lane >= TKF_NHL ? (~PS & TKF_WM) : 0u;
        uint32_t F = R1 & tkf_shr(R1, 1);
        F &= tkf_shr(F, 2);
        F &= tkf_shr(F, 4);
        F &= tkf_shr(F, 8);
        F &= tkf_shr(F, 16);
        F &= wv_up1(F);
        const uint32_t S64 = PS & commit_mask & tkf_shr(F, 1);
        uint32_t LM = 0;
        if (tkf_any(S64)) LM = tkf_ripple(R1, tkf_shl(S64, 1) & R1);
        uint32_t f_lo = TKF_REGION;
        {
            const uint64_t Bm = wv_ballot(lane >= TKF_NHL && PS != 0u);
            if (Bm) {
                const int fl = tk_ctz64(Bm);
                f_lo = (uint32_t)TKF_W * (uint32_t)fl + (uint32_t)__builtin_ctz(wv_readlane(PS, fl));
            }
        }
        uint32_t LMc = 0;
        if (f_lo >= (uint32_t)ca + 64u) {
            const int lo = ca - TKF_W * lane, hi = (int)f_lo - TKF_W * lane;
            LMc = tkf_lowmask32(hi < 0 ? 0 : hi) & ~tkf_lowmask32(lo < 0 ? 0 : lo);
            LM |= LMc;
        }
        const uint32_t ge_cb = ~tkf_lowmask32(cb - TKF_W * lane < 0 ? 0 : cb - TKF_W * lane);
        const bool closed = tkf_any(PS & ge_cb);
        const uint32_t need = LM | tkf_shr(LM, 1);
        uint32_t TG = 0, K2 = 0;
        {
            const uint32_t prevb = wv_dn1(x[TKF_W / 4 - 1]) >> 24;
            uint32_t nb = wv_up1(x[0]) & 0xFFu;
            if (lane == 63) nb = nextb;
            if (need) {
                uint32_t b0 = prevb, b1 = x[0] & 0xFFu;
                for (int k = 0; k < TKF_W; ++k) {
                    const uint32_t b2 = k + 1 < TKF_W ? (x[(k + 1) >> 2] >> (8 * ((k + 1) & 3))) & 0xFFu : nb;
                    if ((need >> k) & 1u) {
                        const uint32_t i3 = b0 | (b1 << 8) | (b2 << 16), i2 = b0 | (b1 << 8);
                        TG |= ((a.t.cut_g3[i3 >> 5] >> (i3 & 31u)) & 1u) << k;
                        K2 |= ((a.t.cut_k2[i2 >> 5] >> (i2 & 31u)) & 1u) << k;
                    }
                    b0 = b1; b1 = b2;
                }
            }
        }
        FS = LM & ~PS & ~K2 & ~TG & ~tkf_shl(TG, 1);
        if (tkf_any(LMc)) {
            const uint32_t win = ((uint32_t)lane == (uint32_t)TKF_NHL || (uint32_t)lane == (uint32_t)TKF_NHL + 1u) ? TKF_WM : 0u;
            if (!tkf_any(FS & LMc & win)) { FS &= ~LMc; LM &= ~LMc; }
        }
        PS |= FS;
        if (closed) own_mask |= LM & ge_cb;
        lds[TKF_L_FS + lane] = FS;
    }

    uint32_t PSown = PS & own_mask;
    uint32_t PSlist = lane >= TKF_NHL ? PS : 0u;
    uint32_t np_all, np_own, pfx_all, pfx_own;
    {
        uint32_t tot;
        const uint32_t pf = tkf_scan_excl((uint32_t)__builtin_popcount(PSlist) | ((uint32_t)__builtin_popcount(PSown) << 16), lane, &tot);
        pfx_all = pf & 0xFFFFu; pfx_own = pf >> 16;
        np_all = tot & 0xFFFFu; np_own = tot >> 16;
    }
    const int npass = np_all > TKF_MAXPIECES ? 2 : 1;
    uint32_t* tmp = WV_KARGS(TkFlatArgs, a).tmp + c * TKF_STRIDE;
    uint32_t* mq = WV_KARGS(TkFlatArgs, a).miss_list + c * TKF_MISSCAP;
    uint32_t E = 0;
    uint32_t base_own = 0;
    uint32_t nm0 = 0, nm1 = 0, nm2 = 0, nm3 = 0;
    uint32_t lane_lo = TKF_NHL, lane_hi = 64;
    auto doc_outputs = [&](bool want_flags, bool anybad) {
        const uint64_t dfirst = fd > 0 ? fd - 1 : 0;
        const auto& ka = WV_KARGS(TkFlatArgs, a);
        for (uint64_t base = dfirst;; base += 64) {
            const uint64_t d = base + (uint64_t)lane;
            int64_t s = INT64_MAX, e = INT64_MAX;
            if (d < ka.n_docs) {
                s = (int64_t)ka.doc_offs[d];
                e = (int64_t)ka.doc_offs[d + 1];
            }
            const bool in = s < c1;
            if (in && s >= c0) {
                const uint32_t p = (uint32_t)(s - r0);
                const uint32_t pl = p >> TKF_LOGW;
                if (npass == 1 || (pl >= lane_lo && pl < lane_hi)) {
                    const uint32_t pi = lds[TKF_L_PFX + pl] + (uint32_t)__builtin_popcount(lds[TKF_L_PS + pl] & ((1u << (p & (TKF_W - 1))) - 1u));
                    ka.lstart[d] = pi < np_own ? list[pi] : base_own + np_own + E;
                }
            }
            if (want_flags && anybad && in && e > c0) {
                const int64_t lo = s > r0 ? s - r0 : 0, hi = e < r1 ? e - r0 : TKF_REGION;
                if (hi > lo) {
                    const uint32_t pl = (uint32_t)lo, ph = (uint32_t)hi;
                    const uint32_t cl = lds[TKF_L_BPFX + (pl >> TKF_LOGW)] + (uint32_t)__builtin_popcount(lds[TKF_L_BAD + (pl >> TKF_LOGW)] & ((1u << (pl & (TKF_W - 1))) - 1u));
                    uint32_t ch;
                    if (ph >= TKF_REGION) ch = lds[TKF_L_BPFX + 63] + (uint32_t)__builtin_popcount(lds[TKF_L_BAD + 63]);
                    else ch = lds[TKF_L_BPFX + (ph >> TKF_LOGW)] + (uint32_t)__builtin_popcount(lds[TKF_L_BAD + (ph >> TKF_LOGW)] & ((1u << (ph & (TKF_W - 1))) - 1u));
                    if (ch > cl) ka.flags[d] = 1u;
                }
            }
            if (wv_ballot(in) != ~0ull) break;
        }
    };
  for (int pass = 0; pass < npass; ++pass) {
    uint32_t sentinel = TKF_REGION;
    if (npass == 2) {
        lane_lo = pass ? 32 : TKF_NHL;
        lane_hi = pass ? 64 : 32;
        const bool mine = (uint32_t)lane >= lane_lo && (uint32_t)lane < lane_hi;
        PSlist = mine ? PS : 0u;
        PSown = PSlist & own_mask;
        uint32_t tot;
        const uint32_t pf = tkf_scan_excl((uint32_t)__builtin_popcount(PSlist) | ((uint32_t)__builtin_popcount(PSown) << 16), lane, &tot);
        pfx_all = pf & 0xFFFFu; pfx_own = pf >> 16;
        np_all = tot & 0xFFFFu; np_own = tot >> 16;
        if (pass == 0) {
            const uint64_t Bm = wv_ballot(lane >= 32 && PS != 0u);
            if (Bm) {
                const int fl = (int)__builtin_ctzll(Bm);
                sentinel = (uint32_t)TKF_W * (uint32_t)fl + (uint32_t)__builtin_ctz(wv_readlane(PS, fl));
            }
        }
    }
    {
        uint32_t w = PSlist, idx = pfx_all;
        while (wv_ballot(w != 0u)) {
            if (w) {
                list[idx++] = (uint16_t)(TKF_W * lane + __builtin_ctz(w));
                w &= w - 1u;
            }
        }
        if (lane == 0) list[np_all] = (uint16_t)sentinel;
    }
    lds[TKF_L_PS + lane] = PSown;
    lds[TKF_L_PFX + lane] = pfx_own;
    wv_lds_sync();

    const uint32_t nbatch = (np_own + 63u) / 64u;
    for (uint32_t j = 0; j < nbatch; ++j) {
        const uint32_t idx = j * 64u + (uint32_t)lane;
        const bool act = idx < np_own;
        uint32_t pos, len;
        if (j + 1u < nbatch) {
            const uint32_t p0 = list[idx], p1 = list[idx + 1u];
            pos = p0;
            len = p1 - p0;
        } else {
            const uint32_t p0 = list[idx < np_all ? idx : np_all], p1 = list[idx < np_all ? idx + 1 : np_all];
            pos = act ? p0 : 0u;
            len = act ? p1 - p0 : 1u;
// ... 3 lines not shown
            const uint32_t* tw = lds + TKF_L_TXT + (pos >> 2);
            const uint32_t t0 = tw[0], t1 = tw[1], t2 = tw[2], t3 = tw[3], t4 = tw[4];
            const uint32_t sh = pos & 3u;
            const uint32_t* km = lds + TKF_L_KM + 4u * (len < 16u ? len : 16u);
            kk[0] = wv_alignbyte(t1, t0, sh) & km[0]; kk[1] = wv_alignbyte(t2, t1, sh) & km[1];
            kk[2] = wv_alignbyte(t3, t2, sh) & km[2]; kk[3] = wv_alignbyte(t4, t3, sh) & km[3];
        }
        uint32_t r = kk[0];
        uint32_t h = 0;
        if (TKF_ABL(a, 1)) {
            r = 7u;
        } else if (TKF_ABL(a, 64)) {
            r = (kk[0] ^ kk[1] ^ kk[2] ^ kk[3]) & 0xFFFFu;
        } else {
            h = tk_key_hash((uint32_t)MODE, kk[0], kk[1], kk[2], kk[3], len);
            if (TKF_ABL(a, 128)) {
                r = h & 0xFFFFu;
            } else if (len - 2u <= 14u) {
                const uint32_t* kc = lds + TKF_L_CONST;
                const uint64_t b8 = (uint64_t)kc[2] | ((uint64_t)kc[3] << 32), b16 = (uint64_t)kc[4] | ((uint64_t)kc[5] << 32);
                r = tk_probe_key_h(wv_global_ptr(b8), TKF_ABL(a, 512) ? kc[0] >> 4 : kc[0], wv_global_ptr(b16), TKF_ABL(a, 512) ? kc[1] >> 4 : kc[1],
                                   h, kk[0], kk[1], kk[2], kk[3], len);
            }
        }
        bool frag = false;
        if (CUT) {
            const uint32_t pe = pos + len;
            frag = act && ((((lds[TKF_L_FS + (pos >> TKF_LOGW)] >> (pos & (TKF_W - 1))) & 1u) != 0u) ||
                           (pe < (uint32_t)TKF_REGION && ((lds[TKF_L_FS + (pe >> TKF_LOGW)] >> (pe & (TKF_W - 1))) & 1u) != 0u));
            if (frag && len >= 2u) r = TK_RANK_MAX;
        }
        bool toolong = false;
        if (wv_ballot(len > 16u)) {
            uint32_t lres = 0;
            bool lopen = false;
            if (len > 64u) {
                lopen = idx + 1u == np_all && sentinel == TKF_REGION && r0 + (int64_t)TKF_REGION < (int64_t)a.n_bytes;
                const bool have_ctl = (lds[TKF_L_CONST + 6] | lds[TKF_L_CONST + 7]) != 0u;
                if (!PAT && have_ctl && (lopen || len <= TKF_LONGCAP) && !(CUT && frag && lopen)) lres = lopen ? TKF_LONGCAP : len;
                else toolong = true;
            } else if (len > 16u && !TKF_ABL(a, 1) && !(CUT && frag)) {
                r = TK_RANK_MAX;
                const uint32_t pb = tk_k64_prebit(h);
                const uint32_t* pre = reinterpret_cast<const uint32_t*>(t.key64_tab + t.key64_mask + 1u);
                const bool maybe = TKF_ABL(a, 64) || TKF_ABL(a, 128) || ((pre[pb >> 5] >> (pb & 31u)) & 1u) != 0u;
                if (maybe) r = tk_probe_key64(t, lds + TKF_L_TXT + (pos >> 2), pos & 3u, len, kk[0], kk[1], kk[2], kk[3]);
            }
            if (toolong) wv_lds_or(lds + TKF_L_BAD + (pos >> TKF_LOGW), 1u << (pos & (TKF_W - 1)));
            if (wv_ballot(lres != 0u)) {
                const bool longp = lres != 0u;
                const bool lmiss = r == TK_RANK_MAX && !toolong && !longp && !TKF_ABL(a, 2);
                uint32_t lslot = base_own + idx + E;
                {
                    uint32_t tot;
                    lslot += tkf_scan_excl(lmiss ? len - 1u : longp ? lres - 1u : 0u, lane, &tot);
                    E += tot;
                }
                {
                    const uint64_t LB = wv_ballot(longp);
                    const int lfirst = tk_ctz64(LB);
                    const uint32_t* ctl = reinterpret_cast<const uint32_t*>(wv_global_ptr((uint64_t)lds[TKF_L_CONST + 6] | ((uint64_t)lds[TKF_L_CONST + 7] << 32)));
                    uint32_t qbase = 0;
                    if (lane == lfirst) qbase = wv_atomic_add(const_cast<uint32_t*>(ctl) + TKC_CTL(TKC_LONG_RECS), (uint32_t)tk_popc64(LB));
                    qbase = wv_shfl(qbase, lfirst);
                    const uint32_t q = qbase + (uint32_t)tk_popc64(LB & tk_lowmask(lane));
                    TkFlatLongRec* recs = reinterpret_cast<TkFlatLongRec*>(const_cast<uint8_t*>(wv_global_ptr((uint64_t)ctl[TKC_CTL(TKC_LONG_CTL)] | ((uint64_t)ctl[TKC_CTL(TKC_LONG_CTL_HI)] << 32))));
                    if (!longp) {
                    } else if (q < ctl[TKC_CTL(TKC_LONG_CTL_CAP)]) {
                        TkFlatLongRec lr;
                        lr.pos = (uint64_t)(r0 + (int64_t)pos); lr.chunk = (uint32_t)c; lr.slot = lslot; lr.len = lopen ? 0u : (CUT && frag ? len | TKF_LREC_FRAG : len); lr.reserved = lres;
                        recs[q] = lr;
                    } else {
                        wv_lds_or(lds + TKF_L_BAD + (pos >> TKF_LOGW), 1u << (pos & (TKF_W - 1)));
                    }
                }
                if (wv_ballot(lmiss)) {
                    const uint32_t cls = (len > 8u ? 1u : 0u) + (len > 16u ? 1u : 0u) + (len > 32u ? 1u : 0u);
                    const uint32_t sh = cls * 8u;
                    uint32_t ctot;
                    const uint32_t before = (tkf_scan_excl(lmiss ? 1u << sh : 0u, lane, &ctot) >> sh) & 0xFFu;
                    if (lmiss) {
                        const uint32_t qb = cls == 0u ? TKF_MISSOFF0 + nm0 : cls == 1u ? TKF_MISSOFF1 + nm1 : cls == 2u ? TKF_MISSOFF2 + nm2 : TKF_MISSOFF3 + nm3;
                        mq[qb + before] = TKF_REC(pos, len, lslot);
                    }
                    nm0 += ctot & 0xFFu;
                    nm1 += (ctot >> 8) & 0xFFu;
                    nm2 += (ctot >> 16) & 0xFFu;
                    nm3 += ctot >> 24;
                }
                wv_lds_sync();
                if (act) {
                    list[idx] = (uint16_t)lslot;
                    if (!lmiss && !longp && !TKF_ABL(a, 4)) tmp[lslot] = r + t.num_special;
                }
                continue;
            }
        }
        const bool miss = r == TK_RANK_MAX && !toolong && !TKF_ABL(a, 2);
        uint32_t slot = base_own + idx + E;
        const uint64_t MB = wv_ballot(miss);
        uint32_t res = len;
        bool mhit = false;
        uint32_t mv0 = 0, mv1 = 0, mv2 = 0, mv4 = 0;
        if (MB) {
            const uint64_t mbase = MEMO ? (uint64_t)wv_first(lds[TKF_L_MEMO + 0]) | ((uint64_t)wv_first(lds[TKF_L_MEMO + 1]) << 32) : 0ull;
            if (MEMO && mbase != 0ull) {
                if (miss && len <= 16u) {
                    const uint32_t ms = tk_memo_slot(h) & lds[TKF_L_MEMO + 2];
                    const tk_u32x4* me = reinterpret_cast<const tk_u32x4*>(wv_global_ptr(mbase) + ((uint64_t)ms << 5));
                    tk_u32x4 ek = me[0], ev = me[1];
                    WV_PIN(ek.x); WV_PIN(ev.x);
                    if ((((ek.x ^ kk[0]) | (ek.y ^ kk[1]) | (ek.z ^ kk[2]) | (ek.w ^ kk[3])) == 0u) && tk_memo_len(ev.w) == len) {
                        mhit = true;
                        res = tk_memo_n(ev.w);
                        mv0 = ev.y; mv1 = ev.z; mv2 = ev.w; mv4 = ev.x;
                    }
                }
                const uint64_t HB = wv_ballot(mhit);
                if (HB && lane == 0) lds[TKF_L_MEMO + 3] += (uint32_t)tk_popc64(HB);
            }
            if ((MB & (MB - 1ull)) == 0ull) {
                const int src = tk_ctz64(MB);
                const uint32_t extra = wv_readlane(res, src) - 1u;
                if (lane > src) slot += extra;
                E += extra;
            } else {
                uint32_t tot;
                slot += tkf_scan_excl(miss ? res - 1u : 0u, lane, &tot);
                E += tot;
            }
            const bool qmiss = MEMO ? miss && !mhit : miss;
            const uint64_t QB = wv_ballot(qmiss);
            if (QB == 0ull) {
            } else if (wv_ballot(qmiss && len > 8u) == 0ull) {
                if (qmiss) mq[TKF_MISSOFF0 + nm0 + (uint32_t)tk_popc64(QB & tk_lowmask(lane))] = TKF_REC(pos, len, slot);
                nm0 += (uint32_t)tk_popc64(QB);
            } else {
                const uint32_t cls = (len > 8u ? 1u : 0u) + (len > 16u ? 1u : 0u) + (len > 32u ? 1u : 0u);
                const uint32_t sh = cls * 8u;
                uint32_t ctot;
                const uint32_t before = (tkf_scan_excl(qmiss ? 1u << sh : 0u, lane, &ctot) >> sh) & 0xFFu;
                if (qmiss) {
                    const uint32_t qb = cls == 0u ? TKF_MISSOFF0 + nm0 : cls == 1u ? TKF_MISSOFF1 + nm1 : cls == 2u ? TKF_MISSOFF2 + nm2 : TKF_MISSOFF3 + nm3;
                    mq[qb + before] = TKF_REC(pos, len, slot);
                }
                nm0 += ctot & 0xFFu;
                nm1 += (ctot >> 8) & 0xFFu;
                nm2 += (ctot >> 16) & 0xFFu;
                nm3 += ctot >> 24;
            }
        }
        wv_lds_sync();
        if (act) {
            list[idx] = (uint16_t)slot;
            if (!miss && !TKF_ABL(a, 4)) tmp[slot] = r + t.num_special;
        }
        if (MEMO && mhit) {
            tmp[slot] = tk_memo_id(mv4, mv0, mv1, mv2, 0u) + t.num_special;
            if (res > 1u) tmp[slot + 1u] = tk_memo_id(mv4, mv0, mv1, mv2, 1u) + t.num_special;
            if (res > 2u) tmp[slot + 2u] = tk_memo_id(mv4, mv0, mv1, mv2, 2u) + t.num_special;
            if (res > 3u) tmp[slot + 3u] = tk_memo_id(mv4, mv0, mv1, mv2, 3u) + t.num_special;
            if (res > 4u) tmp[slot + 4u] = tk_memo_id(mv4, mv0, mv1, mv2, 4u) + t.num_special;
        }
    }
    if (pass + 1 < npass) {
        wv_lds_sync();
        doc_outputs(false, false);
        base_own += np_own;
        wv_lds_sync();
    }
  }
    if (lane == 0) {
        const auto& ka = WV_KARGS(TkFlatArgs, a);
        ka.kcount[c] = base_own + np_own + E;
        ka.miss_count[c] = nm0;
        ka.miss_count[ka.n_chunks + c] = nm1;
        ka.miss_count[2 * ka.n_chunks + c] = nm2;
        ka.miss_count[3 * ka.n_chunks + c] = nm3;
    }

    BAD |= lds[TKF_L_BAD + lane];
    const bool anybad = tkf_any(BAD);
    if (anybad) {
        uint32_t nb;
        const uint32_t bp = tkf_scan_excl((uint32_t)__builtin_popcount(BAD), lane, &nb);
        lds[TKF_L_BAD + lane] = BAD;
        lds[TKF_L_BPFX + lane] = bp;
    }
    wv_lds_sync();
    doc_outputs(true, anybad);
    wv_lds_sync();
    return false;
}

TK_DEV void tk_flat_long_wave(const TkFlatArgs& a, const TkPolyPow& pw, uint32_t q, int lane, uint32_t* scratch) {
    const TkFlatLongRec lr = a.long_recs[q];
    const uint64_t g = lr.pos;
    uint64_t d = a.first_doc[lr.chunk];
    d = d > 0 ? d - 1 : 0;
    while (d + 1 < a.n_docs && a.doc_offs[d + 1] <= g) ++d;
    d = wv_first64(d);
    if (wv_first(a.flags[d]) != 0u) return;
    TkEncodeArgs ea;
    ea.bytes = a.bytes; ea.doc_offs = a.doc_offs; ea.n_docs = a.n_docs; ea.staging = nullptr; ea.counts = nullptr;
    ea.work_counter = nullptr; ea.defer_count = nullptr; ea.defer_list = nullptr; ea.todo_list = nullptr; ea.n_todo = 0; ea.n_todo_dev = nullptr;
    ea.scratch = scratch; ea.scratch_words_per_wave = 0; ea.add_bos = 0; ea.add_eos = 0; ea.split_only = 0; ea.pattern = 0; ea.dbg_ablate = 0;
    ea.dbg_starts = nullptr; ea.dbg_mark = nullptr; ea.long_list = nullptr; ea.long_count = nullptr; ea.long_min = 0; ea.long_lazy_mul = 0; ea.long_force = 0;
    ea.long_jobs = nullptr; ea.long_job_count = nullptr; ea.long_job_cap = 0; ea.t = a.t;
    const uint64_t s1 = wv_first64(a.doc_offs[d + 1]);
    const bool frag = (lr.len & TKF_LREC_FRAG) != 0u;
    const uint32_t rlen = lr.len & ~TKF_LREC_FRAG;
    const uint64_t e = rlen ? g + rlen : wv_first64(tk_match_end(a.t, a.bytes, g, s1));
    const uint32_t len = (uint32_t)(e - g);
    uint32_t* out = a.tmp + (uint64_t)lr.chunk * TKF_STRIDE + lr.slot;
    if (e - g > (uint64_t)lr.reserved) {
        if (lane == 0) {
            if (a.late_list) {
                if (wv_atomic_exch(a.flags + d, 1u) == 0u) a.late_list[wv_atomic_add(a.late_count, 1u)] = (uint32_t)d;
            } else {
                a.flags[d] = 1u;
            }
        }
        return;
    }
    uint32_t cur = 0;
    const uint32_t r = frag ? TK_RANK_MAX : tk_piece_lookup(ea, pw, lane, g, e);
    if (r != TK_RANK_MAX) {
        if (lane == 0) out[0] = r + a.t.num_special;
        cur = 1;
    } else if (a.long_merge128) {
        if (lane == 0) {
            a.long_recs[q].len = len;
            a.long_recs[q].reserved = lr.reserved | (len <= 128u ? 0x80000000u : 0x40000000u);
        }
        return;
    } else {
        tk_piece_merge_coop(ea, lane, g, e, out, cur, scratch);
    }
    for (uint32_t k = cur + (uint32_t)lane; k < lr.reserved; k += 64u) out[k] = TKF_HOLE;
    if (lane == 0) wv_atomic_add(a.holes + d, lr.reserved - cur);
}

TK_DEV void tk_flat_long_coop_wave(const TkFlatArgs& a, uint32_t q, int lane, uint32_t* scratch) {
    TkFlatLongRec lr = a.long_recs[q];
    if (wv_first(lr.reserved & 0x40000000u) == 0u) return;
    lr.reserved &= 0x3FFFFFFFu;
    const uint64_t g = lr.pos;
    uint64_t d = a.first_doc[lr.chunk];
    d = d > 0 ? d - 1 : 0;
    while (d + 1 < a.n_docs && a.doc_offs[d + 1] <= g) ++d;
    d = wv_first64(d);
    uint32_t* out = a.tmp + (uint64_t)lr.chunk * TKF_STRIDE + lr.slot;
    uint32_t cur = 0;
    (void)scratch;
    tk_piece_merge_small(a.t, a.bytes, lane, g, lr.len, out, cur);
    for (uint32_t k = cur + (uint32_t)lane; k < lr.reserved; k += 64u) out[k] = TKF_HOLE;
    if (lane == 0) wv_atomic_add(a.holes + d, lr.reserved - cur);
}

#define TKM_SHORT 16

struct TkMemoLog {
    tk_memo_entry* base;
    uint32_t n, cap;
};
template <bool WIDE>
TK_DEV void tk_merge_items(const TkFlatArgs& a, bool have, uint32_t rec, uint32_t chunk, int lane, uint32_t* mlds, const uint32_t* filt, TkMemoLog* ml = nullptr);

template <bool WIDE>
TK_DEV bool tk_merge_find(const TkFlatArgs& a, uint64_t wave_id, int lane, bool& have_out, uint32_t& rec_out, uint32_t& chunk_out) {
    const uint64_t* prefix = a.miss_prefix;
    const uint64_t n_e = 4 * a.n_chunks;
    const uint64_t first = WIDE ? prefix[2 * a.n_chunks] : 0, total = WIDE ? prefix[3 * a.n_chunks] : prefix[2 * a.n_chunks];
    const uint64_t item0 = first + wave_id * 64;
    have_out = false; rec_out = 0u; chunk_out = 0u;
    if (item0 >= total) return false;
    const uint64_t item = item0 + (uint64_t)lane;
    const bool have = item < total;
    uint64_t cl = 0, pcl = 0;
    {
        uint64_t base = (WIDE ? a.wave_first_wide : a.wave_first)[wave_id];
        uint64_t pbase = prefix[base];
        bool done = !have;
        int windows = 0;
        for (;;) {
            const uint64_t idx = base + 1 + (uint64_t)lane;
            const uint64_t pf = idx <= n_e ? prefix[idx] : ~0ull;
            const uint32_t d = pf <= item0 ? 0u : (pf - item0 > 64 ? 65u : (uint32_t)(pf - item0));
            uint32_t cnt = 0;
            for (uint32_t step = 32; step >= 1; step >>= 1) {
                const uint32_t dm = wv_shfl(d, (int)(cnt + step - 1u));
                if (dm <= (uint32_t)lane) cnt += step;
            }
            const uint32_t d63 = wv_shfl(d, 63);
            if (cnt == 63u && d63 <= (uint32_t)lane) cnt = 64u;
            const uint32_t dprev = wv_shfl(d, cnt ? (int)cnt - 1 : 0);
            if (!done && cnt < 64u) {
                cl = base + cnt;
                pcl = cnt ? item0 + dprev : pbase;
                done = true;
            }
            if (wv_ballot(!done) == 0ull) break;
            pbase = ((uint64_t)wv_shfl((uint32_t)(pf >> 32), 63) << 32) | wv_shfl((uint32_t)pf, 63);
            base += 64;
            if (++windows < 3) continue;
            if (!done) {
                uint64_t lo = base, hi = WIDE ? 3 * a.n_chunks : 2 * a.n_chunks;
                while (hi - lo > 1) {
                    const uint64_t mid = (lo + hi) / 2;
                    if (prefix[mid] <= item) lo = mid; else hi = mid;
                }
                cl = lo;
                pcl = prefix[lo];
                done = true;
            }
            break;
        }
    }
    uint32_t rec = 0;
    uint64_t chunk = 0;
    if (have) {
        const uint64_t k = cl / a.n_chunks;
        chunk = cl - k * a.n_chunks;
        const uint32_t off = k == 0 ? TKF_MISSOFF0 : k == 1 ? TKF_MISSOFF1 : k == 2 ? TKF_MISSOFF2 : TKF_MISSOFF3;
        rec = a.miss_list[chunk * TKF_MISSCAP + off + (item - pcl)];
    }
    have_out = have; rec_out = rec; chunk_out = (uint32_t)chunk;
    return true;
}
template <bool WIDE>
TK_DEV void tk_merge_wave(const TkFlatArgs& a, uint64_t wave_id, int lane, uint32_t* mlds, const uint32_t* filt, TkMemoLog* ml = nullptr) {
    bool have; uint32_t rec, chunk;
    if (!tk_merge_find<WIDE>(a, wave_id, lane, have, rec, chunk)) return;
    tk_merge_items<WIDE>(a, have, rec, chunk, lane, mlds, filt, ml);
}

TK_DEV void tk_merge_items64(const TkFlatArgs& a, bool have, uint32_t rec, uint32_t chunk, int lane, uint32_t* mlds, const uint32_t* filt);
TK_DEV void tk_merge_wave_long3(const TkFlatArgs& a, uint64_t wave_id, int lane, uint32_t* mlds, const uint32_t* filt) {
    const uint64_t* prefix = a.miss_prefix;
    const uint64_t e0 = 3 * a.n_chunks, e1 = 4 * a.n_chunks;
    const uint64_t first = prefix[e0], total = prefix[e1];
    const uint64_t item0 = first + wave_id * 64;
    if (item0 >= total) return;
    const uint64_t item = item0 + (uint64_t)lane;
    const bool have = item < total;
    uint32_t rec = 0;
    uint64_t chunk = 0;
    if (have) {
        uint64_t lo = e0, hi = e1;
        while (hi - lo > 1) {
            const uint64_t mid = (lo + hi) / 2;
            if (prefix[mid] <= item) lo = mid; else hi = mid;
        }
        chunk = lo - e0;
        rec = a.miss_list[chunk * TKF_MISSCAP + TKF_MISSOFF3 + (item - prefix[lo])];
    }
    tk_merge_items64(a, have, rec, (uint32_t)chunk, lane, mlds, filt);
}

#ifndef TKM_COMPACT_MIN
#define TKM_COMPACT_MIN 32
#endif
#define TKM_COMPACT(N) ((N) >= TKM_COMPACT_MIN)
#define TKM_LDS_WORDS(N) (TKM_COMPACT(N) ? ((N) + (N) / 4) * 64 : 2 * (N) * 64)
#ifdef TKM_ABLATE
#define TKM_AB(a, bit) (((a).dbg_ablate & (bit)) != 0)
#else
#define TKM_AB(a, bit) false
#endif
template <int N> struct TkmAlive { typedef uint32_t type; };
template <> struct TkmAlive<64> { typedef uint64_t type; };
template <> struct TkmAlive<128> { typedef unsigned __int128 type; };
template <typename T> TK_DEV T tkm_low(uint32_t n, const T*) { return n >= 8u * (uint32_t)sizeof(T) ? (T)~(T)0 : (T)(((T)1 << n) - (T)1); }
template <typename T> TK_DEV T tkm_bit(uint32_t n, const T*) { return (T)((T)1 << n); }
template <typename T> TK_DEV bool tkm_any(T v) { return v != (T)0; }
template <typename T> TK_DEV T tkm_clear_lowest(T v) { return (T)(v & (v - (T)1)); }
TK_DEV uint32_t tkm_ctz(uint32_t v) { return (uint32_t)__builtin_ctz(v); }
TK_DEV uint32_t tkm_ctz(uint64_t v) { return (uint32_t)__builtin_ctzll(v); }
TK_DEV uint32_t tkm_msb(uint32_t v) { return 31u - (uint32_t)__builtin_clz(v); }
TK_DEV uint32_t tkm_msb(uint64_t v) { return 63u - (uint32_t)__builtin_clzll(v); }
TK_DEV uint32_t tkm_popc(uint32_t v) { return (uint32_t)__builtin_popcount(v); }
TK_DEV uint32_t tkm_popc(uint64_t v) { return (uint32_t)__builtin_popcountll(v); }
TK_DEV uint32_t tkm_ctz(unsigned __int128 v) { const uint64_t lo = (uint64_t)v; return lo ? (uint32_t)__builtin_ctzll(lo) : 64u + (uint32_t)__builtin_ctzll((uint64_t)(v >> 64)); }
TK_DEV uint32_t tkm_msb(unsigned __int128 v) { const uint64_t hi = (uint64_t)(v >> 64); return hi ? 127u - (uint32_t)__builtin_clzll(hi) : 63u - (uint32_t)__builtin_clzll((uint64_t)v); }
TK_DEV uint32_t tkm_popc(unsigned __int128 v) { return (uint32_t)__builtin_popcountll((uint64_t)v) + (uint32_t)__builtin_popcountll((uint64_t)(v >> 64)); }

template <int N>
TK_DEV uint32_t tk_merge_lds(const TkFlatArgs& a, const uint32_t* filt, bool mine, const uint32_t* kk, uint32_t len,
                             uint32_t* out, uint32_t* mlds, int lane, TkMemoLog* ml = nullptr) {
    typedef typename TkmAlive<N>::type alive_t;
    constexpr uint32_t PB = N > 64 ? 7u : N > 32 ? 6u : 5u, PM = (1u << PB) - 1u;
    constexpr uint32_t DEAD = 0x80000000u;
    const TkTablesView& t = a.t;
    constexpr bool C = TKM_COMPACT(N);
    uint32_t* keyc = C ? mlds + lane : mlds + N * 64 + lane;
    uint32_t* bytc = mlds + N * 64 + lane;
    uint32_t* tokc = mlds + lane;
    const uint32_t n = mine ? len : 0u;
    if (C) {
#pragma unroll
        for (int q = 0; q < N / 4; ++q) bytc[q * 64] = kk[q];
    }
#pragma unroll
    for (int i = 0; i < N; ++i) {
        const uint32_t b = (kk[i >> 2] >> (8 * (i & 3))) & 0xFFu;
        const uint32_t b1 = i + 1 < N ? (kk[(i + 1) >> 2] >> (8 * ((i + 1) & 3))) & 0xFFu : 0u;
        uint32_t key = 0xFFFFFFFFu;
        if ((uint32_t)(i + 1) < n && !TKM_AB(a, 2048)) {
            const uint32_t r = t.pair2[b | (b1 << 8)];
            if (r != TK_RANK_MAX) key = (r << PB) | (uint32_t)i;
        }
        if (!C) tokc[i * 64] = b;
        keyc[i * 64] = key;
    }
    alive_t alive = tkm_low(n, (const alive_t*)nullptr);
    auto tok_at = [&](uint32_t x, alive_t al) -> uint32_t {
        if (!C) return tokc[x * 64u];
        const bool multi = x + 1u < n && !tkm_any((alive_t)(al & tkm_bit(x + 1u < (uint32_t)N ? x + 1u : 0u, (const alive_t*)nullptr)));
        const uint32_t v = multi ? keyc[(x + 1u) * 64u] : bytc[(x >> 2) * 64u];
        return multi ? v & ~DEAD : (v >> (8u * (x & 3u))) & 0xFFu;
    };
    bool active = mine && !TKM_AB(a, 1024);
    while (wv_ballot(active)) {
        if (active) {
            uint32_t best = 0xFFFFFFFFu;
#pragma unroll
            for (int i = 0; i < N - 1; ++i) {
                const uint32_t k = keyc[i * 64];
                best = k < best ? k : best;
            }
            if (best >= DEAD) {
                active = false;
            } else {
                const uint32_t bi = best & PM, rank = best >> PB;
                const alive_t above = alive & ~tkm_low(bi + 1u, (const alive_t*)nullptr);
                const uint32_t j = tkm_ctz(above);
                const alive_t above2 = tkm_clear_lowest(above);
                const alive_t below = alive & tkm_low(bi, (const alive_t*)nullptr);
                const bool has_next = tkm_any(above2), has_prev = tkm_any(below);
                const uint32_t k = has_next ? tkm_ctz(above2) : 0u;
                const uint32_t p = has_prev ? tkm_msb(below) : 0u;
                const uint32_t tn = tok_at(k, alive), tp = tok_at(p, alive);
                alive = alive & ~tkm_bit(j, (const alive_t*)nullptr);
                keyc[j * 64] = 0xFFFFFFFFu;
                if (C) keyc[(bi + 1u) * 64] = DEAD | rank;
                else tokc[bi * 64] = rank;
                uint32_t r_next = TK_RANK_MAX, r_prev = TK_RANK_MAX;
                tk_probe_pair_x2f(t, filt, has_next, rank, tn, has_prev, tp, rank, r_next, r_prev);
                keyc[bi * 64] = r_next == TK_RANK_MAX ? 0xFFFFFFFFu : ((r_next << PB) | bi);
                if (has_prev) keyc[p * 64] = r_prev == TK_RANK_MAX ? 0xFFFFFFFFu : ((r_prev << PB) | p);
            }
        }
    }
    const uint32_t np = tkm_popc(alive);
    if (!C && ml != nullptr) {
        bool ins = mine && np <= TK_MEMO_MAXIDS;
        uint32_t k[4] = {0u, 0u, 0u, 0u};
        tk_memo_entry* slot = nullptr;
        if (wv_ballot(ins) && ml->n < ml->cap) {
            if (ins) {
#pragma unroll
                for (int q = 0; q < 4; ++q) {
                    const int keep = (int)len - 4 * q;
                    k[q] = (q < N / 4 && keep > 0) ? (kk[q < N / 4 ? q : 0] & (keep >= 4 ? 0xFFFFFFFFu : ((1u << (8 * keep)) - 1u))) : 0u;
                }
                slot = a.memo_tab + (tk_memo_slot(tk_key_hash(t.key_hash_mode, k[0], k[1], k[2], k[3], len)) & a.memo_mask);
                if (a.memo_probe == 0u) {
                    const uint32_t cw = slot->w4;
                    if (cw != 0u && (cw & TK_MEMO_TAG) == 0u) ins = false;
                }
            }
        }
        const uint64_t IB = wv_ballot(ins);
        if (IB && ml->n < ml->cap) {
            const uint32_t at = ml->n + (uint32_t)tk_popc64(IB & tk_lowmask(lane));
            if (ins && at < ml->cap) {
                uint32_t r5[5] = {0u, 0u, 0u, 0u, 0u};
                alive_t rem = alive;
#pragma unroll
                for (int q = 0; q < 5; ++q) {
                    if ((uint32_t)q < np) r5[q] = tokc[tkm_ctz(rem) * 64u];
                    rem = tkm_clear_lowest(rem);
                }
                uint32_t v[3], w4;
                tk_memo_pack(r5, np, len, &w4, v);
                tk_memo_entry* w = ml->base + at;
                wv_store16(w->k, k[0], k[1], k[2], k[3]);
                wv_store16(&w->w4, w4, v[0], v[1], v[2]);
                slot->w4 = (uint32_t)(w - a.memo_log);
            }
            const uint32_t nn = ml->n + (uint32_t)tk_popc64(IB);
            ml->n = nn < ml->cap ? nn : ml->cap;
        }
    }
    if (mine && !TKM_AB(a, 256)) {
        alive_t rem = alive;
#pragma unroll
        for (int q0 = 0; q0 < N; q0 += 4) {
            uint32_t v[4];
#pragma unroll
            for (int q = 0; q < 4; ++q) {
                const uint32_t pos = tkm_any(rem) ? tkm_ctz(rem) : 0u;
                const uint32_t id = tok_at(pos, alive) + t.num_special;
                v[q] = (uint32_t)(q0 + q) < np ? id : TKF_HOLE;
                rem = tkm_clear_lowest(rem);
            }
            if ((uint32_t)q0 + 4u <= len) {
                wv_store16(out + q0, v[0], v[1], v[2], v[3]);
            } else {
                if ((uint32_t)q0 < len) out[q0] = v[0];
                if ((uint32_t)q0 + 1u < len) out[q0 + 1] = v[1];
                if ((uint32_t)q0 + 2u < len) out[q0 + 2] = v[2];
            }
        }
    }
    return mine ? len - np : 0u;
}

TK_DEV void tk_merge_holes(const TkFlatArgs& a, bool have, uint32_t holes, uint32_t chunk, int64_t g, int lane) {
    if (wv_ballot(have && holes != 0u) && !TKM_AB(a, 512)) {
        uint64_t d = 0;
        if (have) {
            d = a.first_doc[chunk];
            d = d > 0 ? d - 1 : 0;
            for (;;) {
                const uint64_t i1 = d + 1 < a.n_docs ? d + 1 : a.n_docs, i2 = d + 2 < a.n_docs ? d + 2 : a.n_docs;
                const uint64_t i3 = d + 3 < a.n_docs ? d + 3 : a.n_docs, i4 = d + 4 < a.n_docs ? d + 4 : a.n_docs;
                uint64_t o1 = a.doc_offs[i1], o2 = a.doc_offs[i2], o3 = a.doc_offs[i3], o4 = a.doc_offs[i4];
                const uint32_t cnt = ((int64_t)o1 <= g ? 1u : 0u) + ((int64_t)o2 <= g ? 1u : 0u) + ((int64_t)o3 <= g ? 1u : 0u) + ((int64_t)o4 <= g ? 1u : 0u);
                d += cnt;
                if (cnt < 4u) break;
            }
        }
        const uint32_t key = have ? (uint32_t)d : 0xFFFFFFFFu;
        const uint32_t kprev = wv_shfl(key, lane > 0 ? lane - 1 : 0), knext = wv_shfl(key, lane < 63 ? lane + 1 : 63);
        const bool head = lane == 0 || kprev != key, tail = lane == 63 || knext != key;
        const uint64_t HEADS = wv_ballot(head);
        const uint32_t P = wv_scan_incl_u32(have ? holes : 0u);
        const int start = tk_msb64(HEADS & (tk_lowmask(lane) | (1ull << lane)));
        const uint32_t before = wv_shfl(P, start > 0 ? start - 1 : 0);
        const uint32_t sum = P - (start > 0 ? before : 0u);
        if (have && tail && sum) wv_atomic_add(a.holes + d, sum);
    }
}

TK_DEV void tk_merge_items64(const TkFlatArgs& a, bool have, uint32_t rec, uint32_t chunk, int lane, uint32_t* mlds, const uint32_t* filt) {
    const uint32_t pos = TKF_REC_POS(rec), len = TKF_REC_LEN(rec), slot = TKF_REC_SLOT(rec);
    const int64_t g = (int64_t)chunk * TKF_COMMIT - TKF_HL + (int64_t)pos;
    uint32_t* out = a.tmp + (uint64_t)chunk * TKF_STRIDE + slot;
    uint32_t kk[16];
    for (int q = 0; q < 16; ++q) kk[q] = 0u;
    if (have) {
        if (g + 64 <= (int64_t)a.n_bytes) {
            wv_load16(a.bytes + g, kk);
            wv_load16(a.bytes + g + 16, kk + 4);
            wv_load16(a.bytes + g + 32, kk + 8);
            wv_load16(a.bytes + g + 48, kk + 12);
        } else {
            for (uint32_t q = 0; q < len; ++q) kk[q >> 2] |= (uint32_t)a.bytes[g + q] << (8 * (q & 3));
        }
    }
    uint32_t holes = 0;
    if (wv_ballot(have)) holes = tk_merge_lds<64>(a, filt, have, kk, len, out, mlds, lane);
    tk_merge_holes(a, have, holes, chunk, g, lane);
}

template <int N>
TK_DEV void tk_merge_long_wave(const TkFlatArgs& a, uint64_t wave_id, int lane, uint32_t* mlds, const uint32_t* filt) {
    const uint64_t n = *a.long_count < a.long_cap ? *a.long_count : a.long_cap;
    const uint64_t item = wave_id * 64 + (uint64_t)lane;
    if (wave_id * 64 >= n) return;
    TkFlatLongRec lr;
    lr.pos = 0; lr.chunk = 0; lr.slot = 0; lr.len = 0; lr.reserved = 0;
    if (item < n) lr = a.long_recs[item];
    const bool have = (lr.reserved & 0x80000000u) != 0u && lr.len <= (uint32_t)N && lr.len > (uint32_t)N / 2u;
    lr.reserved &= 0x3FFFFFFFu;
    if (wv_ballot(have) == 0ull) return;
    const int64_t g = (int64_t)lr.pos;
    uint32_t* out = a.tmp + (uint64_t)lr.chunk * TKF_STRIDE + lr.slot;
    uint32_t kk[N / 4];
    for (int q = 0; q < N / 4; ++q) kk[q] = 0u;
    if (have) {
        if (g + N <= (int64_t)a.n_bytes) {
#pragma unroll
            for (int q = 0; q < N / 16; ++q) wv_load16(a.bytes + g + 16 * q, kk + 4 * q);
        } else {
            for (uint32_t q = 0; q < lr.len; ++q) kk[q >> 2] |= (uint32_t)a.bytes[g + q] << (8 * (q & 3));
        }
    }
    uint32_t holes = tk_merge_lds<N>(a, filt, have, kk, lr.len, out, mlds, lane);
    if (have) {
        for (uint32_t k = lr.len; k < lr.reserved; ++k) out[k] = TKF_HOLE;
        holes += lr.reserved - lr.len;
    }
    tk_merge_holes(a, have, holes, lr.chunk, g, lane);
}

template <bool WIDE>
TK_DEV void tk_merge_items(const TkFlatArgs& a, bool have, uint32_t rec, uint32_t chunk, int lane, uint32_t* mlds, const uint32_t* filt, TkMemoLog* ml) {
    const TkTablesView& t = a.t;
    const uint32_t pos = TKF_REC_POS(rec), len = TKF_REC_LEN(rec), slot = TKF_REC_SLOT(rec);
    const int64_t g = (int64_t)chunk * TKF_COMMIT - TKF_HL + (int64_t)pos;
    uint32_t* out = a.tmp + (uint64_t)chunk * TKF_STRIDE + slot;
    uint32_t holes = 0;

    {
        const uint32_t cap = WIDE ? 32u : TKM_SHORT;
        const bool inregs = have && len <= cap;
        uint32_t kk[WIDE ? 8 : 4];
        for (int q = 0; q < (WIDE ? 8 : 4); ++q) kk[q] = 0u;
        if (inregs) {
            if (g + (int64_t)cap <= (int64_t)a.n_bytes) {
                wv_load16(a.bytes + g, kk);
                if (WIDE) wv_load16(a.bytes + g + 16, kk + 4);
            } else {
                for (uint32_t q = 0; q < len; ++q) kk[q >> 2] |= (uint32_t)a.bytes[g + q] << (8 * (q & 3));
            }
        }
        if (!WIDE) {
            const bool s8 = inregs && len <= 8u, s16 = inregs && len > 8u;
            if (wv_ballot(s8)) holes += tk_merge_lds<8>(a, filt, s8, kk, len, out, mlds, lane, ml);
            if (wv_ballot(s16)) holes += tk_merge_lds<16>(a, filt, s16, kk, len, out, mlds, lane, ml);
        } else {
            if (wv_ballot(inregs)) holes += tk_merge_lds<32>(a, filt, inregs, kk, len, out, mlds, lane);
        }
    }

    uint64_t LONGM = wv_ballot(have && len > (WIDE ? 32u : TKM_SHORT));
    while (LONGM) {
        const int src = tk_ctz64(LONGM);
        LONGM &= LONGM - 1ull;
        const uint32_t plen = wv_shfl(len, src);
        const uint32_t glo = wv_shfl((uint32_t)g, src), ghi = wv_shfl((uint32_t)((uint64_t)g >> 32), src);
        const int64_t pg = (int64_t)(((uint64_t)ghi << 32) | glo);
        const uint32_t pchunk = wv_shfl(chunk, src), pslot = wv_shfl(slot, src);
        uint32_t* pout = a.tmp + (uint64_t)pchunk * TKF_STRIDE + pslot;
        const int pe = (int)plen;
        const bool inmiss = lane < pe;
        const uint32_t b0 = inmiss ? (uint32_t)a.bytes[pg + lane] : 0u;
        const uint32_t b1 = wv_up1(b0);
        uint64_t A = wv_ballot(inmiss);
        uint32_t tok = b0;
        uint32_t prank = TK_RANK_MAX;
        if (inmiss && lane + 1 < pe) prank = t.pair2[b0 | (b1 << 8)];
        for (int round = 0; round < 64; ++round) {
            const uint32_t key = prank == TK_RANK_MAX ? 0xFFFFFFFFu : ((prank << 6) | (uint32_t)lane);
            const uint32_t segmin = wv_min_u32(key);
            if (segmin == 0xFFFFFFFFu) break;
            const bool winner = key == segmin;
            const uint64_t Wm = wv_ballot(winner);
            const bool alive = tk_bit(A, lane);
            const uint64_t below = A & tk_lowmask(lane);
            const bool dead = alive && below && tk_bit(Wm, tk_msb64(below));
            const uint64_t Dm = wv_ballot(dead);
            A &= ~Dm;
            if (winner) tok = prank;
            if (dead) prank = TK_RANK_MAX;
            const uint64_t z = lane < 63 ? (A >> (lane + 1)) : 0ull;
            const int na = z ? lane + 1 + tk_ctz64(z) : 64;
            const bool has_next = na < pe;
            const uint32_t tn = wv_shfl(tok, na < 64 ? na : lane);
            const bool need = tk_bit(A, lane) && (winner || (has_next && tk_bit(Wm, na)));
            if (need) prank = has_next ? tk_probe_pair_f(t, filt, tok, tn) : TK_RANK_MAX;
        }
        const uint32_t k = (uint32_t)tk_popc64(A);
        if (inmiss && tk_bit(A, lane)) pout[tk_popc64(A & tk_lowmask(lane))] = tok + t.num_special;
        if (inmiss && (uint32_t)lane >= k) pout[lane] = TKF_HOLE;
        if (lane == src) holes = plen - k;
    }

    tk_merge_holes(a, have, holes, chunk, g, lane);
}

TK_DEV bool tk_memo_log_live(const uint32_t* counts, uint32_t per_wave, uint32_t i) { return i % per_wave < counts[i / per_wave]; }
TK_DEV uint32_t tk_memo_slot_of(const tk_memo_entry& r, uint32_t key_hash_mode, uint32_t mask) {
    return tk_memo_slot(tk_key_hash(key_hash_mode, r.k[0], r.k[1], r.k[2], r.k[3], tk_memo_len(r.v[2]))) & mask;
}
TK_DEV void tk_memo_commit_one(tk_memo_entry* tab, const tk_memo_entry* log, uint32_t i, uint32_t key_hash_mode, uint32_t mask) {
    const tk_memo_entry r = log[i];
    tk_memo_entry* w = tab + tk_memo_slot_of(r, key_hash_mode, mask);
    if (w->w4 == i) {
        wv_store16(w->k, r.k[0], r.k[1], r.k[2], r.k[3]);
        wv_store16(&w->w4, r.w4, r.v[0], r.v[1], r.v[2]);
    }
}

#endif
```

tekken-rs_amd/csrc/tk_pipeline.cpp:

```cpp
#include <algorithm>

#include "tk_ctx.h"

static TkCallKnobs call_knobs() {
    TkCallKnobs k;
    k.log = getenv("TK_DEBUG_LOG") != nullptr;
    k.marks = getenv("TK_DEBUG_MARKS") != nullptr;
    k.skip_pass2 = getenv("TK_DEBUG_SKIP_PASS2") != nullptr;
    if (const char* ll = getenv("TK_MEMO_LOG_LOG2")) { const int v = atoi(ll); if (v >= 8 && v <= 24) k.memo_log_log2 = v; }
#ifdef TK_ABLATE
    if (const char* ab = getenv("TK_DEBUG_ABLATE")) k.ablate = atoi(ab);
#endif
    return k;
}

static uint64_t cu_count(const tk_ctx* c) {
    int cus = 256;
    (void)hipDeviceGetAttribute(&cus, hipDeviceAttributeMultiprocessorCount, c->device);
    return (uint64_t)cus;
}

TkEncodeArgs encode_args(tk_ctx* c, const uint8_t* d_bytes, const uint64_t* d_offs, uint64_t n_docs, int add_bos, int add_eos) {
    TkEncodeArgs a;
    memset(&a, 0, sizeof(a));
// ... 174 lines not shown
static int memo_prepare(tk_ctx* c, TkFlatArgs& fa, hipStream_t s, uint64_t n_bytes) {
    TkKnobs& k = c->knobs;
    c->memo_active_last = false;
    if (k.memo_log2 == 0) return TK_OK;
    if (k.memo_policy == 0 && n_bytes < (1u << 20)) return TK_OK;
    if (k.memo_policy == 0 && c->memo_pause) { --c->memo_pause; return TK_OK; }
    const size_t bytes = ((size_t)1 << k.memo_log2) * sizeof(tk_memo_entry);
    if (c->memo_have_log2 != k.memo_log2) {
        c->t_memo.release();
        if (c->t_memo.reserve(bytes) != hipSuccess) {
            (void)hipGetLastError();
            k.memo_log2 = 0; c->memo_have_log2 = 0;
            return TK_OK;
        }
        TK_HIP(c, hipMemsetAsync(c->t_memo.p, 0, bytes, s));
        c->memo_have_log2 = k.memo_log2;
        c->memo_epoch = 0;
    }
    if (c->memo_epoch >= 0xFFFFFFF0u) {
        TK_HIP(c, hipMemsetAsync(c->t_memo.p, 0, bytes, s));
        c->memo_epoch = 0;
    }
    const uint32_t log_waves = (uint32_t)cu_count(c) * 16u;
    const uint32_t log_log2 = c->call.memo_log_log2 ? (uint32_t)c->call.memo_log_log2 : k.memo_log2 > 23 ? 21 : k.memo_log2 - 2;
    const uint32_t log_cap = 1u << log_log2;
    const uint32_t per_wave = log_cap / log_waves > 0 ? log_cap / log_waves : 1u;
    if (c->t_memo_log.reserve((size_t)per_wave * log_waves * sizeof(tk_memo_entry) + (size_t)log_waves * 4) != hipSuccess) {
        (void)hipGetLastError();
        c->t_memo.release();
        k.memo_log2 = 0; c->memo_have_log2 = 0;
        return TK_OK;
    }
    fa.memo_tab = (tk_memo_entry*)c->t_memo.p;
    fa.memo_mask = (1u << k.memo_log2) - 1u;
    fa.memo_log = (tk_memo_entry*)c->t_memo_log.p;
    fa.memo_log_counts = (uint32_t*)(fa.memo_log + (size_t)per_wave * log_waves);
    fa.memo_log_per_wave = per_wave;
    fa.memo_log_waves = log_waves;
    TK_HIP(c, hipMemsetAsync(fa.memo_log_counts, 0, (size_t)log_waves * 4, s));
    fa.memo_epoch = ++c->memo_epoch;
    fa.memo_probe = c->memo_epoch > 1 ? 1 : 0;
    fa.memo_hits = c->ctr(TKC_MEMO_HITS);
    c->memo_active_last = true;
    return TK_OK;
}
static void memo_account(tk_ctx* c, const uint32_t* final_ctr, uint64_t n_bytes) {
    c->memo_hits_last = c->memo_lookups_last = 0;
    if (!c->memo_active_last) return;
    c->memo_hits_last = final_ctr[TKC_MEMO_HITS];
    c->memo_lookups_last = (uint64_t)final_ctr[TKC_MEMO_HITS] + final_ctr[TKC_NARROW_LEFT];
    c->memo_hits_total += c->memo_hits_last;
    c->memo_lookups_total += c->memo_lookups_last;
    if (c->knobs.memo_policy != 0 || c->memo_epoch < 2 || n_bytes < (1u << 20)) return;
    const bool pays = c->memo_hits_last * 10 >= c->memo_lookups_last * 3 && c->memo_hits_last * 160 >= n_bytes;
    if (pays) c->memo_low_streak = 0;
    else if (++c->memo_low_streak >= 2) { c->memo_pause = 30; c->memo_low_streak = 0; }
}

struct FlatRun {
    tk_ctx* c;
    const uint8_t* d_bytes;
    const uint64_t* d_offs;
    uint64_t n_docs, n_bytes, n_chunks;
    int add_bos, add_eos;
    hipStream_t s, sb;
    bool serial;
    uint64_t wf_narrow;
    uint64_t total;
    TkFlatArgs fa;
};

static int flat_reserve(FlatRun& r) {
    tk_ctx* c = r.c;
    const uint64_t n_chunks = r.n_chunks, n_docs = r.n_docs;
    TK_HIP(c, c->f_first.reserve((n_chunks + 1) * 4));
    TK_HIP(c, c->f_tmp.reserve((n_chunks * TKF_STRIDE + 64) * 4));
    TK_HIP(c, c->f_lstart.reserve((n_docs + 1) * 4));
    TK_HIP(c, c->f_flags.reserve(2 * (n_docs + 1) * 4));
    TK_HIP(c, c->f_todo.reserve((n_docs + 1) * 4));
    TK_HIP(c, c->f_miss.reserve((n_chunks * TKF_MISSCAP + 64) * 4));
    TK_HIP(c, c->f_mcnt.reserve((5 * n_chunks + 1) * 4));
    TK_HIP(c, c->f_mpfx.reserve((5 * n_chunks + 2) * 8));
    TK_HIP(c, c->f_info.reserve((n_docs + 1) * 16));
    r.wf_narrow = n_chunks * (TKF_MISSOFF2 / 64 + 1) + 64;
    const uint64_t wf_wide = n_chunks * ((TKF_MISSCAP - TKF_MISSOFF2) / 64 + 1) + 64;
    TK_HIP(c, c->f_wfirst.reserve((r.wf_narrow + wf_wide) * 4));
    TK_HIP(c, c->counts.reserve((n_docs + 1) * 4));
    TK_HIP(c, c->out_offs.reserve((n_docs + 1) * 8));
    const uint64_t scan_n = n_docs > 5 * n_chunks ? n_docs : 5 * n_chunks;
    TK_HIP(c, c->block_sums.reserve((scan_n / 2048 + 4) * 8));
    return TK_OK;
}

static void flat_args(FlatRun& r) {
    tk_ctx* c = r.c;
    TkFlatArgs& fa = r.fa;
    memset(&fa, 0, sizeof(fa));
    fa.bytes = r.d_bytes;
    fa.doc_offs = r.d_offs;
    fa.n_docs = r.n_docs;
    fa.n_bytes = r.n_bytes;
    fa.n_chunks = r.n_chunks;
    fa.first_doc = (const uint32_t*)c->f_first.p;
    fa.tmp = (uint32_t*)c->f_tmp.p;
    fa.kcount = (uint32_t*)c->f_mcnt.p + 4 * r.n_chunks;
    fa.lstart = (uint32_t*)c->f_lstart.p;
    fa.flags = (uint32_t*)c->f_flags.p;
    fa.miss_list = (uint32_t*)c->f_miss.p;
    fa.miss_count = (uint32_t*)c->f_mcnt.p;
    fa.miss_prefix = (const uint64_t*)c->f_mpfx.p;
    fa.holes = (uint32_t*)c->f_flags.p + (r.n_docs + 1);
    fa.wave_first = (uint32_t*)c->f_wfirst.p;
    fa.wave_first_wide = (uint32_t*)c->f_wfirst.p + r.wf_narrow;
    fa.t = c->dview;
    fa.pattern = c->pattern;
    fa.dbg_ablate = c->call.ablate;
}

static int flat_control_words(FlatRun& r) {
    tk_ctx* c = r.c;
    TkFlatArgs& fa = r.fa;
    if (c->knobs.no_flat_long) return TK_OK;
    TK_HIP(c, c->f_long.reserve((r.n_bytes / 65 + 1024) * sizeof(TkFlatLongRec)));
    fa.long_recs = (TkFlatLongRec*)c->f_long.p;
    fa.long_count = c->ctr(TKC_LONG_RECS);
    fa.long_cap = (uint32_t)std::min<uint64_t>(c->f_long.cap / sizeof(TkFlatLongRec), 0xFFFFFFF0ull);
    fa.long_ctl = c->ctr(TKC_LONG_CTL);
    if (c->long_ctl_ptr != c->f_long.p || c->long_ctl_cap != fa.long_cap) {
        const uint64_t pv = (uint64_t)reinterpret_cast<uintptr_t>(c->f_long.p);
        const uint32_t words[] = {(uint32_t)pv, (uint32_t)(pv >> 32), fa.long_cap};
        TK_HIP(c, hipMemcpyAsync(c->ctr(TKC_LONG_CTL), words, sizeof(words), hipMemcpyHostToDevice, r.s));
        TK_HIP(c, hipStreamSynchronize(r.s));
        c->long_ctl_ptr = c->f_long.p;
        c->long_ctl_cap = fa.long_cap;
    }
    void* want_cut = nullptr;
    if (!c->knobs.no_flat_cut && c->pattern == 0) {
        TK_HIP(c, c->f_cut.reserve((r.n_chunks + 1) * 4));
        want_cut = c->f_cut.p;
        fa.cut_list = (uint32_t*)c->f_cut.p;
        fa.cut_count = c->ctr(TKC_CUT_CHUNKS);
    }
    if (c->cut_ctl_ptr != want_cut) {
        const uint64_t pv = (uint64_t)reinterpret_cast<uintptr_t>(want_cut);
        const uint32_t words[] = {(uint32_t)pv, (uint32_t)(pv >> 32)};
        TK_HIP(c, hipMemcpyAsync(c->ctr(TKC_CUT_CTL), words, sizeof(words), hipMemcpyHostToDevice, r.s));
        TK_HIP(c, hipStreamSynchronize(r.s));
        c->cut_ctl_ptr = want_cut;
    }
    return TK_OK;
}

static int flat_fork_todo(FlatRun& r) {
    tk_ctx* c = r.c;
    if (!r.serial) {
        TK_HIP(c, hipEventRecord(c->ev_b[0], r.s));
        TK_HIP(c, hipStreamWaitEvent(r.sb, c->ev_b[0], 0));
    }
    TK_HIP(c, tk_launch_flat_todo(r.fa.flags, r.d_offs, r.n_docs, (uint32_t*)c->f_todo.p, c->ctr(TKC_TODO), c->ctr(TKC_TODO_MAXLEN), r.sb));
    if (!r.serial) {
        TK_HIP(c, hipMemcpyAsync(c->h_pin + TKC_EARLY_MIRROR, c->ctr(TKC_WORK), TKC_EARLY_WORDS * 4, hipMemcpyDeviceToHost, r.sb));
        TK_HIP(c, hipEventRecord(c->ev_b[1], r.sb));
    }
    return TK_OK;
}

static int flat_finish(FlatRun& r, int final_pass, bool wait) {
    tk_ctx* c = r.c;
    const TkFlatArgs& fa = r.fa;
    const uint32_t extra = (uint32_t)((r.add_bos ? 1 : 0) + (r.add_eos ? 1 : 0));
    const uint64_t* d_P = (const uint64_t*)c->f_mpfx.p + 4 * r.n_chunks;
    TK_HIP(c, tk_launch_flat_counts(r.d_offs, r.n_docs, r.n_bytes, r.n_chunks, d_P, fa.lstart, fa.flags, fa.holes, extra,
                                    (uint32_t*)c->counts.p, c->f_info.p, final_pass, c->ctr(TKC_HANDED_BACK), r.s));
    TK_HIP(c, tk_launch_scan((const uint32_t*)c->counts.p, r.n_docs, (uint64_t*)c->out_offs.p, (uint64_t*)c->block_sums.p, r.s));
    TK_HIP(c, tk_launch_flat_assemble(r.n_docs, c->f_info.p, fa.kcount, (const uint64_t*)c->out_offs.p, fa.tmp,
                                      (const uint32_t*)c->staging.p, (uint32_t*)c->out_ids.p, c->host.bos_id,
                                      c->host.eos_id, r.add_bos, r.add_eos, (uint64_t*)c->ctr(TKC_TOTAL),
                                      final_pass ? nullptr : c->ctr(TKC_HANDED_BACK), r.s));
    TK_HIP(c, hipEventRecord(c->ev[2], r.s));
    TK_HIP(c, hipMemcpyAsync(c->h_pin, c->ctr(TKC_WORK), TKC_FINAL_WORDS * 4, hipMemcpyDeviceToHost, r.s));
    if (wait) {
        TK_HIP(c, hipStreamSynchronize(r.s));
        ++c->host_syncs;
        memcpy(&r.total, c->h_pin + TKC_TOTAL, 8);
    }
    return TK_OK;
}
// ... 59 lines not shown
}

static int flat_complete(FlatRun& r, const uint32_t* early) {
    tk_ctx* c = r.c;
    const uint32_t n_todo = early[TKC_TODO];
    uint32_t n_lrec = early[TKC_LONG_RECS];
    const uint64_t maxlen = early[TKC_TODO_MAXLEN];
    c->n_cut_chunks = early[TKC_CUT_CHUNKS];
    c->n_flagged = n_todo;
    c->n_long_docs = 0;
    c->n_long_recs = 0;
    if (c->call.log) fprintf(stderr, "[tk] flat: docs=%llu chunks=%llu handed back=%u (longest %llu bytes) long-piece records=%u cut chunks=%u\n",
                             (unsigned long long)r.n_docs, (unsigned long long)r.n_chunks, n_todo, (unsigned long long)maxlen, n_lrec, early[TKC_CUT_CHUNKS]);
    if (n_todo == 0 && n_lrec == 0) {
        if (!r.serial) {
            TK_HIP(c, hipStreamSynchronize(r.s));
            ++c->host_syncs;
            memcpy(&r.total, c->h_pin + TKC_TOTAL, 8);
        }
        return TK_OK;
    }
    TK_HIP(c, c->staging.reserve((r.n_bytes + 2 * r.n_docs + 64) * 4));
    TK_HIP(c, c->defer_list.reserve((r.n_docs + 1) * 4));
    TkEncodeArgs a = encode_args(c, r.d_bytes, r.d_offs, r.n_docs, r.add_bos, r.add_eos);
    a.pattern = c->pattern;
    if (n_lrec > r.fa.long_cap) n_lrec = r.fa.long_cap;
    c->n_long_recs = n_lrec;
    int rc = flat_enqueue_tail(r, a, n_lrec, n_todo, maxlen);
    if (rc != TK_OK || (rc = flat_finish(r, 1, true)) != TK_OK) return rc;
    if (c->h_pin[TKC_PASS2_SPARE] == TKC_OVERFLOW) { c->err = "internal: the long-piece job list overflowed"; return TK_ERR_RUNTIME; }
    c->n_long_docs = c->pattern == 1 ? n_todo : c->h_pin[TKC_DEFERRED];
    c->n_round_docs += n_todo && c->knobs.long_min ? c->h_pin[TKC_LONG_JOBS] : 0;
    const uint32_t n_late = n_lrec ? c->h_pin[TKC_LATE] : 0;
    return n_late ? flat_redo_late(r, a, n_late) : TK_OK;
}

static int run_pipeline_flat(tk_ctx* c, const uint8_t* d_bytes, const uint64_t* d_offs, uint64_t n_docs, uint64_t n_bytes,
                             int add_bos, int add_eos, hipStream_t s, uint64_t* n_ids) {
    const bool serial = c->knobs.serial_tail;
    FlatRun r = {c, d_bytes, d_offs, n_docs, n_bytes, (n_bytes + TKF_COMMIT - 1) / TKF_COMMIT, add_bos, add_eos,
                 s, serial ? s : (hipStream_t)c->stream_b, serial, 0, 0, {}};
    int rc = flat_reserve(r);
    if (rc != TK_OK) return rc;
    flat_args(r);
    if ((rc = flat_control_words(r)) != TK_OK) return rc;
    TK_HIP(c, c->out_ids.reserve((n_bytes + 2 * n_docs + 64) * 4));
    if ((rc = memo_prepare(c, r.fa, s, n_bytes)) != TK_OK) return rc;
    TK_HIP(c, hipEventRecord(c->ev[3], s));
    TK_HIP(c, tk_launch_flat_firstdoc(d_offs, n_docs, r.n_chunks, (uint32_t*)c->f_first.p, r.fa.flags, r.fa.holes, c->ctr(TKC_WORK), s));
    TK_HIP(c, hipEventRecord(c->ev[0], s));
    TK_HIP(c, tk_launch_flat(r.fa, s));
    TK_HIP(c, hipEventRecord(c->ev[1], s));
    if (r.fa.dbg_ablate & 24) {
        TK_HIP(c, hipEventRecord(c->ev[2], s));
        TK_HIP(c, hipStreamSynchronize(s));
        (void)hipEventElapsedTime(&c->encode_ms, c->ev[0], c->ev[1]);
        (void)hipEventElapsedTime(&c->pipeline_ms, c->ev[3], c->ev[2]);
        c->n_flagged = 0;
        *n_ids = 0;
        return TK_OK;
    }
    c->host_syncs = 0;
    struct JoinStreams {
        hipStream_t a, b;
        bool armed;
        ~JoinStreams() { if (armed) { (void)hipStreamSynchronize(b); (void)hipStreamSynchronize(a); } }
    } join_guard{s, r.sb, true};
    if ((rc = flat_fork_todo(r)) != TK_OK) return rc;
    TK_HIP(c, tk_launch_scan(r.fa.miss_count, 5 * r.n_chunks, (uint64_t*)c->f_mpfx.p, (uint64_t*)c->block_sums.p, s));
    TK_HIP(c, tk_launch_merge(r.fa, c->ctr(TKC_NARROW_LEFT), s));
    TK_HIP(c, hipEventRecord(c->ev[4], s));
    if ((rc = flat_finish(r, 0, r.serial)) != TK_OK) return rc;
    const uint32_t* early = c->h_pin;
    if (!r.serial) {
        TK_HIP(c, hipEventSynchronize(c->ev_b[1]));
        ++c->host_syncs;
        early = c->h_pin + TKC_EARLY_MIRROR;
    }
    if ((rc = flat_complete(r, early)) != TK_OK) return rc;
    (void)hipEventElapsedTime(&c->encode_ms, c->ev[0], c->ev[1]);
    (void)hipEventElapsedTime(&c->pipeline_ms, c->ev[3], c->ev[2]);
    (void)hipEventElapsedTime(&c->merge_ms, c->ev[1], c->ev[4]);
    memo_account(c, c->h_pin, n_bytes);
    *n_ids = r.total;
    join_guard.armed = false;
    return TK_OK;
}

static int run_pipeline_seq(tk_ctx* c, const uint8_t* d_bytes, const uint64_t* d_offs, uint64_t n_docs, uint64_t n_bytes,
                            int add_bos, int add_eos, hipStream_t s, uint64_t* n_ids) {
    int rc = reserve_doc_buffers(c, n_docs, n_bytes);
    if (rc != TK_OK) return rc;
    TkEncodeArgs a = encode_args(c, d_bytes, d_offs, n_docs, add_bos, add_eos);
    a.pattern = 1;
    c->n_flagged = 0;
    c->n_long_docs = n_docs;
    uint64_t total = 0;
    TK_HIP(c, hipEventRecord(c->ev[0], s));
    TK_HIP(c, hipEventRecord(c->ev[3], s));
    if (n_docs) {
        TK_HIP(c, tk_launch_iota((uint32_t*)c->defer_list.p, n_docs, s));
        if ((rc = run_pass2(c, a, d_offs, (uint32_t)n_docs, s, 8192)) != TK_OK) return rc;
    }
    TK_HIP(c, hipEventRecord(c->ev[1], s));
    if ((rc = scan_compact(c, a, s)) != TK_OK) return rc;
    TK_HIP(c, hipMemcpyAsync(&total, (uint64_t*)c->out_offs.p + n_docs, 8, hipMemcpyDeviceToHost, s));
    TK_HIP(c, hipStreamSynchronize(s));
    (void)hipEventElapsedTime(&c->encode_ms, c->ev[0], c->ev[1]);
    (void)hipEventElapsedTime(&c->pipeline_ms, c->ev[0], c->ev[2]);
    *n_ids = total;
    return TK_OK;
}

int run_pipeline(tk_ctx* c, const uint8_t* d_bytes, const uint64_t* d_offs, uint64_t n_docs, uint64_t n_bytes, int add_bos,
                 int add_eos, hipStream_t s, uint64_t* n_ids) {
    c->call = call_knobs();
    if (c->pattern == 1 && c->knobs.pipeline_forced == 2) return run_pipeline_seq(c, d_bytes, d_offs, n_docs, n_bytes, add_bos, add_eos, s, n_ids);
    c->use_flat = c->knobs.pipeline_forced != 2;
    if (c->use_flat) return run_pipeline_flat(c, d_bytes, d_offs, n_docs, n_bytes, add_bos, add_eos, s, n_ids);
    c->n_flagged = 0;
    return run_pipeline_doc(c, d_bytes, d_offs, n_docs, n_bytes, add_bos, add_eos, s, n_ids);
}
```

Before: 389,100.

## Record miss keys and per-chunk doc boundaries during encode for reuse in merge

The encode pass now saves the packed key bytes of each missed piece into a per-chunk key buffer. It also stores a compact record of the first few document starts in each chunk. The merge pass reads keys from that buffer instead of reloading raw input bytes, and resolves hole document indices from the record instead of searching doc offsets. A vectorised tail store for hole fill is added as well. All three paths are on by default through a miss_records knob set to 7. The trade is extra global writes and buffers in encode in exchange for fewer scattered reads in merge, with a fallback counter for keys that did not fit.

Result: no change. 393,700 (median of 6 runs) (+1.2%).

```diff
diff --git a/include/tekken_hip.h b/include/tekken_hip.h
--- a/include/tekken_hip.h
+++ b/include/tekken_hip.h
@@ -52,6 +52,7 @@
 uint64_t tk_long_piece_records(const tk_ctx* ctx);
 uint64_t tk_cut_chunks(const tk_ctx* ctx);
 uint64_t tk_last_host_syncs(const tk_ctx* ctx);
+uint64_t tk_miss_keys_fallback(const tk_ctx* ctx);
 
 int tk_ctx_set_memo(tk_ctx* ctx, int log2_entries, int policy);
 int tk_ctx_memo_clear(tk_ctx* ctx);
diff --git a/tekken-rs_amd/__init__.py b/tekken-rs_amd/__init__.py
--- a/tekken-rs_amd/__init__.py
+++ b/tekken-rs_amd/__init__.py
@@ -182,6 +182,9 @@
     if hasattr(L, "tk_cut_chunks"):
         L.tk_cut_chunks.restype = ctypes.c_uint64
         L.tk_cut_chunks.argtypes = [vp]
+    if hasattr(L, "tk_miss_keys_fallback"):
+        L.tk_miss_keys_fallback.restype = ctypes.c_uint64
+        L.tk_miss_keys_fallback.argtypes = [vp]
     L.tk_encode_batch_device.restype = ctypes.c_int
     L.tk_encode_batch_device.argtypes = [vp, vp, vp, ctypes.c_uint64, ctypes.c_uint64, ctypes.c_int, ctypes.c_int, vp,
                                          ctypes.POINTER(vp), ctypes.POINTER(vp), ctypes.POINTER(ctypes.c_uint64)]
@@ -985,7 +988,8 @@
     def last_stats(self):
         a, b = ctypes.c_uint64(0), ctypes.c_uint64(0)
         lib().tk_last_stats(self._h, ctypes.byref(a), ctypes.byref(b))
-        return {"long_docs": int(a.value), "handed_back": int(b.value)}
+        return {"long_docs": int(a.value), "handed_back": int(b.value),
+                "miss_keys_fallback": int(lib().tk_miss_keys_fallback(self._h)) if hasattr(lib(), "tk_miss_keys_fallback") else 0}
 
     def split_docs(self, docs):
         data, offs = pack_docs(docs)
diff --git a/tekken-rs_amd/csrc/tk_capi.cpp b/tekken-rs_amd/csrc/tk_capi.cpp
--- a/tekken-rs_amd/csrc/tk_capi.cpp
+++ b/tekken-rs_amd/csrc/tk_capi.cpp
@@ -135,6 +135,7 @@
     if (const char* lf = getenv("TK_LONG_FORCE")) k.long_force = (uint32_t)atoi(lf);
     if (const char* ml = getenv("TK_MEMO_LOG2")) { const int v = atoi(ml); k.memo_log2 = v <= 0 ? 0u : (uint32_t)(v < 10 ? 10 : v > 26 ? 26 : v); }
     if (const char* mp = getenv("TK_MEMO_POLICY")) k.memo_policy = strcmp(mp, "always") == 0 ? 1 : 0;
+    if (const char* mr = getenv("TK_MISS_RECORDS")) k.miss_records = (uint32_t)atoi(mr) & 7u;
     if (const char* pl = getenv("TK_PIPELINE"))
         k.pipeline_forced = strcmp(pl, "doc") == 0 ? 2 : strcmp(pl, "flat") == 0 ? 1 : 0;
 }
@@ -281,6 +282,7 @@
 extern "C" uint64_t tk_long_piece_records(const tk_ctx* c) { return c ? c->n_long_recs : 0; }
 extern "C" uint64_t tk_cut_chunks(const tk_ctx* c) { return c ? c->n_cut_chunks : 0; }
 extern "C" uint64_t tk_last_host_syncs(const tk_ctx* c) { return c ? c->host_syncs : 0; }
+extern "C" uint64_t tk_miss_keys_fallback(const tk_ctx* c) { return c ? c->miss_keys_fallback_last : 0; }
 
 extern "C" int tk_last_stats(const tk_ctx* c, uint64_t* n_long_docs, uint64_t* reserved) {
     if (!c) return TK_ERR_INVALID_ARG;
diff --git a/tekken-rs_amd/csrc/tk_counters.h b/tekken-rs_amd/csrc/tk_counters.h
--- a/tekken-rs_amd/csrc/tk_counters.h
+++ b/tekken-rs_amd/csrc/tk_counters.h
@@ -24,6 +24,7 @@
     TKC_CUT_CTL_HI = 20,
     TKC_MEMO_HITS = 24,
     TKC_NARROW_LEFT = 25,
+    TKC_MISS_KEYS_FALLBACK = 26,
 
     TKC_CLEARED = 16,
     TKC_EARLY_WORDS = 16,
@@ -36,7 +37,7 @@
 #define TKC_OVERFLOW 0xDEADu
 
 static_assert(TKC_LONG_CTL >= TKC_CLEARED && TKC_CUT_CTL_HI < TKC_MEMO_HITS, "the control words lie outside what the pre-pass clears");
-static_assert(TKC_TODO_MAXLEN < TKC_EARLY_WORDS && TKC_NARROW_LEFT < TKC_FINAL_WORDS && TKC_FINAL_WORDS <= TKC_DEVICE_WORDS, "copies hold what the host reads");
+static_assert(TKC_TODO_MAXLEN < TKC_EARLY_WORDS && TKC_MISS_KEYS_FALLBACK < TKC_FINAL_WORDS && TKC_FINAL_WORDS <= TKC_DEVICE_WORDS, "copies hold what the host reads");
 static_assert(TKC_FINAL_WORDS <= TKC_EARLY_MIRROR && TKC_EARLY_MIRROR + TKC_EARLY_WORDS <= TKC_PIN_WORDS, "both copies fit h_pin, apart");
 static_assert(TKC_LONG_CTL_CAP == TKC_LONG_CTL + 2 && TKC_CUT_CTL == TKC_LONG_CTL + 3 && TKC_CUT_CTL_HI == TKC_CUT_CTL + 1, "one block of control words");
 
diff --git a/tekken-rs_amd/csrc/tk_ctx.h b/tekken-rs_amd/csrc/tk_ctx.h
--- a/tekken-rs_amd/csrc/tk_ctx.h
+++ b/tekken-rs_amd/csrc/tk_ctx.h
@@ -70,6 +70,7 @@
     uint32_t memo_log2 = 24;
     int memo_policy = 0;
     int pipeline_forced = 0;
+    uint32_t miss_records = 7;
 };
 struct TkCallKnobs {
     bool log = false;
@@ -133,6 +134,9 @@
     DevBuf f_first, f_tmp, f_lstart, f_flags, f_todo, f_miss, f_mcnt, f_mpfx, f_wfirst, f_info;
     DevBuf f_long;
     DevBuf f_cut;
+    DevBuf f_mkeys, f_drec;
+    uint32_t miss_keys_seen = 0;
+    uint64_t miss_keys_fallback_last = 0;
     DevBuf f_late;
     DevBuf scratch_rec;
     void* long_ctl_ptr = nullptr;
diff --git a/tekken-rs_amd/csrc/tk_flat.hip b/tekken-rs_amd/csrc/tk_flat.hip
--- a/tekken-rs_amd/csrc/tk_flat.hip
+++ b/tekken-rs_amd/csrc/tk_flat.hip
@@ -128,7 +128,9 @@
     ml.base = a.memo_log ? a.memo_log + wave * a.memo_log_per_wave : nullptr;
     ml.n = 0u;
     ml.cap = a.memo_log && wave < a.memo_log_waves ? a.memo_log_per_wave : 0u;
-    for (uint64_t w = wave; w * 64 < total; w += n_waves) tk_merge_wave<false>(a, w, wv_lane(), mlds, TKM_FILTER ? wlds : nullptr, a.memo_log ? &ml : nullptr);
+    uint32_t nokey = 0u;
+    for (uint64_t w = wave; w * 64 < total; w += n_waves) tk_merge_wave<false>(a, w, wv_lane(), mlds, TKM_FILTER ? wlds : nullptr, a.memo_log ? &ml : nullptr, &nokey);
+    if (nokey != 0u && a.miss_keys_fallback && wv_lane() == 0) wv_atomic_add(a.miss_keys_fallback, nokey);
     if (a.memo_log && wave < a.memo_log_waves && wv_lane() == 0) a.memo_log_counts[wave] = ml.n;
 }
 
diff --git a/tekken-rs_amd/csrc/tk_flat_args.h b/tekken-rs_amd/csrc/tk_flat_args.h
--- a/tekken-rs_amd/csrc/tk_flat_args.h
+++ b/tekken-rs_amd/csrc/tk_flat_args.h
@@ -24,6 +24,15 @@
 #define TKF_REC_LEN(rec) (((rec) >> TKF_POSBITS) & 127u)
 #define TKF_REC_SLOT(rec) ((rec) >> (TKF_POSBITS + 7))
 #define TKF_HOLE 0xFFFFFFFFu
+#define TKF_KEYCAP0 32u
+#define TKF_KEYCAP1 32u
+#define TKF_KEYOFF1 (2u * TKF_KEYCAP0)
+#define TKF_KEYSTRIDE (TKF_KEYOFF1 + 4u * TKF_KEYCAP1)
+
+#define TKF_DREC_N 6u
+#define TKF_DREC_NONE 0xFFFu
+#define TKF_DREC_FIELD 0xFFFu
+#define TKF_DREC_CNT_SHIFT 28
 
 struct TkFlatLongRec {
     uint64_t pos;
@@ -40,6 +49,10 @@
     const uint64_t* doc_offs;
     uint64_t n_docs, n_bytes, n_chunks;
     const uint32_t* first_doc;
+    uint32_t* doc_rec;
+    uint32_t* miss_keys;
+    uint32_t* miss_keys_fallback;
+    uint32_t tail_vec;
     uint32_t* tmp;
     uint32_t* kcount;
     uint32_t* lstart;
diff --git a/tekken-rs_amd/csrc/tk_flat_impl.h b/tekken-rs_amd/csrc/tk_flat_impl.h
--- a/tekken-rs_amd/csrc/tk_flat_impl.h
+++ b/tekken-rs_amd/csrc/tk_flat_impl.h
@@ -362,6 +362,14 @@
 
 TK_DEV uint32_t tkf_lowmask32(int n) { return n >= 32 ? 0xFFFFFFFFu : ((1u << n) - 1u); }
 
+TK_DEV void tkf_put_key(uint32_t* mk, uint32_t cls, uint32_t j, const uint32_t* kk) {
+    if (cls == 0u) {
+        if (j < TKF_KEYCAP0) *reinterpret_cast<uint64_t*>(mk + 2u * j) = (uint64_t)kk[0] | ((uint64_t)kk[1] << 32);
+    } else if (cls == 1u && j < TKF_KEYCAP1) {
+        wv_store16(mk + TKF_KEYOFF1 + 4u * j, kk[0], kk[1], kk[2], kk[3]);
+    }
+}
+
 #ifdef TK_ABLATE
 #define TKF_ABL(a, bit) (DBG && ((a).dbg_ablate & (bit)))
 #else
@@ -566,7 +574,19 @@
             const bool in = s < r1;
             if (in) wv_lds_or(lds + TKF_L_DS + ((s - r0) >> TKF_LOGW), 1u << ((s - r0) & (TKF_W - 1)));
             if (s == r1) starts_at_r1 = true;
-            if (wv_ballot(in) != ~0ull) break;
+            const uint64_t IN = wv_ballot(in);
+            if (base == fd) {
+                uint32_t* dr = ka.doc_rec;
+                if (dr != nullptr) {
+                    const uint32_t v = in ? (uint32_t)(s - r0) : TKF_DREC_NONE;
+                    const uint32_t v2 = v | (wv_up1(v) << 16);
+                    const uint32_t nin = (uint32_t)tk_popc64(IN);
+                    const uint32_t w1 = wv_readlane(v2, 0), w2 = wv_readlane(v2, 2);
+                    const uint32_t w3 = wv_readlane(v2, 4) | ((nin > TKF_DREC_N ? TKF_DREC_N + 1u : nin) << TKF_DREC_CNT_SHIFT);
+                    if (lane == 0) wv_store16(dr + 4 * c, (uint32_t)fd, w1, w2, w3);
+                }
+            }
+            if (IN != ~0ull) break;
         }
         starts_at_r1 = wv_ballot(starts_at_r1) != 0ull;
     }
@@ -706,8 +726,7 @@
     }
     const int npass = np_all > TKF_MAXPIECES ? 2 : 1;
     uint32_t* tmp = WV_KARGS(TkFlatArgs, a).tmp + c * TKF_STRIDE;
-    uint32_t* mq = WV_KARGS(TkFlatArgs, a).miss_list + c * TKF_MISSCAP;
-    uint32_t E = 0;
+    uint32_t* mq = WV_KARGS(TkFlatArgs, a).miss_list + c * TKF_MISSCAP;    uint32_t E = 0;
     uint32_t base_own = 0;
     uint32_t nm0 = 0, nm1 = 0, nm2 = 0, nm3 = 0;
     uint32_t lane_lo = TKF_NHL, lane_hi = 64;
@@ -877,6 +896,8 @@
                     if (lmiss) {
                         const uint32_t qb = cls == 0u ? TKF_MISSOFF0 + nm0 : cls == 1u ? TKF_MISSOFF1 + nm1 : cls == 2u ? TKF_MISSOFF2 + nm2 : TKF_MISSOFF3 + nm3;
                         mq[qb + before] = TKF_REC(pos, len, lslot);
+                        uint32_t* mk = WV_KARGS(TkFlatArgs, a).miss_keys;
+                        if (mk != nullptr) tkf_put_key(mk + c * TKF_KEYSTRIDE, cls, (cls == 0u ? nm0 : nm1) + before, kk);
                     }
                     nm0 += ctot & 0xFFu;
                     nm1 += (ctot >> 8) & 0xFFu;
@@ -926,9 +947,15 @@
             }
             const bool qmiss = MEMO ? miss && !mhit : miss;
             const uint64_t QB = wv_ballot(qmiss);
+            uint32_t* mk = QB ? WV_KARGS(TkFlatArgs, a).miss_keys : nullptr;
+            if (mk != nullptr) mk += c * TKF_KEYSTRIDE;
             if (QB == 0ull) {
             } else if (wv_ballot(qmiss && len > 8u) == 0ull) {
-                if (qmiss) mq[TKF_MISSOFF0 + nm0 + (uint32_t)tk_popc64(QB & tk_lowmask(lane))] = TKF_REC(pos, len, slot);
+                if (qmiss) {
+                    const uint32_t qj = nm0 + (uint32_t)tk_popc64(QB & tk_lowmask(lane));
+                    mq[TKF_MISSOFF0 + qj] = TKF_REC(pos, len, slot);
+                    if (mk != nullptr) tkf_put_key(mk, 0u, qj, kk);
+                }
                 nm0 += (uint32_t)tk_popc64(QB);
             } else {
                 const uint32_t cls = (len > 8u ? 1u : 0u) + (len > 16u ? 1u : 0u) + (len > 32u ? 1u : 0u);
@@ -938,6 +965,7 @@
                 if (qmiss) {
                     const uint32_t qb = cls == 0u ? TKF_MISSOFF0 + nm0 : cls == 1u ? TKF_MISSOFF1 + nm1 : cls == 2u ? TKF_MISSOFF2 + nm2 : TKF_MISSOFF3 + nm3;
                     mq[qb + before] = TKF_REC(pos, len, slot);
+                    if (mk != nullptr) tkf_put_key(mk, cls, (cls == 0u ? nm0 : nm1) + before, kk);
                 }
                 nm0 += ctot & 0xFFu;
                 nm1 += (ctot >> 8) & 0xFFu;
@@ -1060,15 +1088,15 @@
     uint32_t n, cap;
 };
 template <bool WIDE>
-TK_DEV void tk_merge_items(const TkFlatArgs& a, bool have, uint32_t rec, uint32_t chunk, int lane, uint32_t* mlds, const uint32_t* filt, TkMemoLog* ml = nullptr);
+TK_DEV void tk_merge_items(const TkFlatArgs& a, bool have, uint32_t rec, uint32_t chunk, uint32_t ord, int lane, uint32_t* mlds, const uint32_t* filt, TkMemoLog* ml = nullptr, uint32_t* nokey = nullptr);
 
 template <bool WIDE>
-TK_DEV bool tk_merge_find(const TkFlatArgs& a, uint64_t wave_id, int lane, bool& have_out, uint32_t& rec_out, uint32_t& chunk_out) {
+TK_DEV bool tk_merge_find(const TkFlatArgs& a, uint64_t wave_id, int lane, bool& have_out, uint32_t& rec_out, uint32_t& chunk_out, uint32_t& ord_out) {
     const uint64_t* prefix = a.miss_prefix;
     const uint64_t n_e = 4 * a.n_chunks;
     const uint64_t first = WIDE ? prefix[2 * a.n_chunks] : 0, total = WIDE ? prefix[3 * a.n_chunks] : prefix[2 * a.n_chunks];
     const uint64_t item0 = first + wave_id * 64;
-    have_out = false; rec_out = 0u; chunk_out = 0u;
+    have_out = false; rec_out = 0u; chunk_out = 0u; ord_out = 0u;
     if (item0 >= total) return false;
     const uint64_t item = item0 + (uint64_t)lane;
     const bool have = item < total;
@@ -1121,13 +1149,14 @@
         rec = a.miss_list[chunk * TKF_MISSCAP + off + (item - pcl)];
     }
     have_out = have; rec_out = rec; chunk_out = (uint32_t)chunk;
+    ord_out = have ? (uint32_t)(item - pcl) : 0u;
     return true;
 }
 template <bool WIDE>
-TK_DEV void tk_merge_wave(const TkFlatArgs& a, uint64_t wave_id, int lane, uint32_t* mlds, const uint32_t* filt, TkMemoLog* ml = nullptr) {
-    bool have; uint32_t rec, chunk;
-    if (!tk_merge_find<WIDE>(a, wave_id, lane, have, rec, chunk)) return;
-    tk_merge_items<WIDE>(a, have, rec, chunk, lane, mlds, filt, ml);
+TK_DEV void tk_merge_wave(const TkFlatArgs& a, uint64_t wave_id, int lane, uint32_t* mlds, const uint32_t* filt, TkMemoLog* ml = nullptr, uint32_t* nokey = nullptr) {
+    bool have; uint32_t rec, chunk, ord;
+    if (!tk_merge_find<WIDE>(a, wave_id, lane, have, rec, chunk, ord)) return;
+    tk_merge_items<WIDE>(a, have, rec, chunk, ord, lane, mlds, filt, ml, nokey);
 }
 
 TK_DEV void tk_merge_items64(const TkFlatArgs& a, bool have, uint32_t rec, uint32_t chunk, int lane, uint32_t* mlds, const uint32_t* filt);
@@ -1290,6 +1319,7 @@
     }
     if (mine && !TKM_AB(a, 256)) {
         alive_t rem = alive;
+        const bool tail_vec = WV_KARGS(TkFlatArgs, a).tail_vec != 0u;
 #pragma unroll
         for (int q0 = 0; q0 < N; q0 += 4) {
             uint32_t v[4];
@@ -1302,6 +1332,8 @@
             }
             if ((uint32_t)q0 + 4u <= len) {
                 wv_store16(out + q0, v[0], v[1], v[2], v[3]);
+            } else if (tail_vec && (uint32_t)q0 < len && len >= 4u && np + 4u <= len) {
+                wv_store16(out + (len - 4u), TKF_HOLE, TKF_HOLE, TKF_HOLE, TKF_HOLE);
             } else {
                 if ((uint32_t)q0 < len) out[q0] = v[0];
                 if ((uint32_t)q0 + 1u < len) out[q0 + 1] = v[1];
@@ -1315,9 +1347,23 @@
 TK_DEV void tk_merge_holes(const TkFlatArgs& a, bool have, uint32_t holes, uint32_t chunk, int64_t g, int lane) {
     if (wv_ballot(have && holes != 0u) && !TKM_AB(a, 512)) {
         uint64_t d = 0;
-        if (have) {
+        bool search = have;
+        const uint32_t* doc_rec = WV_KARGS(TkFlatArgs, a).doc_rec;
+        if (have && doc_rec != nullptr) {
+            uint32_t dr[4];
+            wv_load16(reinterpret_cast<const uint8_t*>(doc_rec + 4 * (uint64_t)chunk), dr);
+            const uint32_t p = (uint32_t)(g - ((int64_t)chunk * TKF_COMMIT - TKF_HL));
+            const uint32_t cnt = ((dr[1] & TKF_DREC_FIELD) <= p ? 1u : 0u) + (((dr[1] >> 16) & TKF_DREC_FIELD) <= p ? 1u : 0u) +
+                                 ((dr[2] & TKF_DREC_FIELD) <= p ? 1u : 0u) + (((dr[2] >> 16) & TKF_DREC_FIELD) <= p ? 1u : 0u) +
+                                 ((dr[3] & TKF_DREC_FIELD) <= p ? 1u : 0u) + (((dr[3] >> 16) & TKF_DREC_FIELD) <= p ? 1u : 0u);
+            const uint64_t dn = (uint64_t)dr[0] + cnt;
+            d = dn > 0 ? dn - 1 : 0;
+            search = cnt == TKF_DREC_N && (dr[3] >> TKF_DREC_CNT_SHIFT) > TKF_DREC_N;
+        } else if (have) {
             d = a.first_doc[chunk];
             d = d > 0 ? d - 1 : 0;
+        }
+        if (search) {
             for (;;) {
                 const uint64_t i1 = d + 1 < a.n_docs ? d + 1 : a.n_docs, i2 = d + 2 < a.n_docs ? d + 2 : a.n_docs;
                 const uint64_t i3 = d + 3 < a.n_docs ? d + 3 : a.n_docs, i4 = d + 4 < a.n_docs ? d + 4 : a.n_docs;
@@ -1392,7 +1438,7 @@
 }
 
 template <bool WIDE>
-TK_DEV void tk_merge_items(const TkFlatArgs& a, bool have, uint32_t rec, uint32_t chunk, int lane, uint32_t* mlds, const uint32_t* filt, TkMemoLog* ml) {
+TK_DEV void tk_merge_items(const TkFlatArgs& a, bool have, uint32_t rec, uint32_t chunk, uint32_t ord, int lane, uint32_t* mlds, const uint32_t* filt, TkMemoLog* ml, uint32_t* nokey) {
     const TkTablesView& t = a.t;
     const uint32_t pos = TKF_REC_POS(rec), len = TKF_REC_LEN(rec), slot = TKF_REC_SLOT(rec);
     const int64_t g = (int64_t)chunk * TKF_COMMIT - TKF_HL + (int64_t)pos;
@@ -1404,7 +1450,22 @@
         const bool inregs = have && len <= cap;
         uint32_t kk[WIDE ? 8 : 4];
         for (int q = 0; q < (WIDE ? 8 : 4); ++q) kk[q] = 0u;
-        if (inregs) {
+        bool stored = false;
+        const uint32_t* miss_keys = WIDE ? nullptr : WV_KARGS(TkFlatArgs, a).miss_keys;
+        if (!WIDE && miss_keys != nullptr) {
+            const uint32_t* mk = miss_keys + (uint64_t)chunk * TKF_KEYSTRIDE;
+            if (inregs && len <= 8u && ord < TKF_KEYCAP0) {
+                const uint64_t k01 = *reinterpret_cast<const uint64_t*>(mk + 2u * ord);
+                kk[0] = (uint32_t)k01; kk[1] = (uint32_t)(k01 >> 32);
+                stored = true;
+            } else if (inregs && len > 8u && ord < TKF_KEYCAP1) {
+                wv_load16(reinterpret_cast<const uint8_t*>(mk + TKF_KEYOFF1 + 4u * ord), kk);
+                stored = true;
+            }
+            const uint64_t FB = wv_ballot(inregs && !stored);
+            if (nokey != nullptr) *nokey += (uint32_t)tk_popc64(FB);
+        }
+        if (inregs && !stored) {
             if (g + (int64_t)cap <= (int64_t)a.n_bytes) {
                 wv_load16(a.bytes + g, kk);
                 if (WIDE) wv_load16(a.bytes + g + 16, kk + 4);
diff --git a/tekken-rs_amd/csrc/tk_pipeline.cpp b/tekken-rs_amd/csrc/tk_pipeline.cpp
--- a/tekken-rs_amd/csrc/tk_pipeline.cpp
+++ b/tekken-rs_amd/csrc/tk_pipeline.cpp
@@ -280,6 +280,8 @@
     TK_HIP(c, c->f_mcnt.reserve((5 * n_chunks + 1) * 4));
     TK_HIP(c, c->f_mpfx.reserve((5 * n_chunks + 2) * 8));
     TK_HIP(c, c->f_info.reserve((n_docs + 1) * 16));
+    if (c->knobs.miss_records & 1u) TK_HIP(c, c->f_mkeys.reserve((n_chunks * TKF_KEYSTRIDE + 64) * 4));
+    if (c->knobs.miss_records & 2u) TK_HIP(c, c->f_drec.reserve((n_chunks + 1) * 16));
     r.wf_narrow = n_chunks * (TKF_MISSOFF2 / 64 + 1) + 64;
     const uint64_t wf_wide = n_chunks * ((TKF_MISSCAP - TKF_MISSOFF2) / 64 + 1) + 64;
     TK_HIP(c, c->f_wfirst.reserve((r.wf_narrow + wf_wide) * 4));
@@ -300,7 +302,10 @@
     fa.n_bytes = r.n_bytes;
     fa.n_chunks = r.n_chunks;
     fa.first_doc = (const uint32_t*)c->f_first.p;
-    fa.tmp = (uint32_t*)c->f_tmp.p;
+    if (c->knobs.miss_records & 1u) { fa.miss_keys = (uint32_t*)c->f_mkeys.p; fa.miss_keys_fallback = c->ctr(TKC_MISS_KEYS_FALLBACK); }
+    if (c->knobs.miss_records & 2u) fa.doc_rec = (uint32_t*)c->f_drec.p;
+    fa.tail_vec = (c->knobs.miss_records & 4u) ? 1u : 0u;
+    fa.tmp =(uint32_t*)c->f_tmp.p;
     fa.kcount = (uint32_t*)c->f_mcnt.p + 4 * r.n_chunks;
     fa.lstart = (uint32_t*)c->f_lstart.p;
     fa.flags = (uint32_t*)c->f_flags.p;
@@ -526,6 +531,8 @@
     (void)hipEventElapsedTime(&c->pipeline_ms, c->ev[3], c->ev[2]);
     (void)hipEventElapsedTime(&c->merge_ms, c->ev[1], c->ev[4]);
     memo_account(c, c->h_pin, n_bytes);
+    c->miss_keys_fallback_last = (uint32_t)(c->h_pin[TKC_MISS_KEYS_FALLBACK] - c->miss_keys_seen);
+    c->miss_keys_seen = c->h_pin[TKC_MISS_KEYS_FALLBACK];
     *n_ids = r.total;
     join_guard.armed = false;
     return TK_OK;
```
